# pangenome/smoothxg

Hardware: AMD Instinct MI355X
Metric: POA blocks/sec (+ DP cells/sec) on 1000-block synthetic (higher is better)
Workload: dtype int16

## Files before the change

### include/sxg_poa.h

```cpp
#ifndef SXG_POA_H
#define SXG_POA_H
#include <stdint.h>

#ifdef __cplusplus
extern "C" {
#endif

#define SXG_POA_ABI_VERSION 5

#define SXG_MODE_LOCAL 0
#define SXG_MODE_GLOBAL 1
#define SXG_ORDER_SPOA 0x10

#define SXG_OK 0
#define SXG_E_INVALID (-1)
#define SXG_E_NODEVICE (-2)
#define SXG_E_NOMEM (-3)
#define SXG_E_BLOCK (-4)
#define SXG_NOT_ROOT 1

#define SXG_ST_OK 0
#define SXG_ST_ROWS_OVERFLOW 1
#define SXG_ST_POOL_OVERFLOW 2
#define SXG_ST_TBX_OVERFLOW 3
// ... 44 lines not shown
    int32_t *edge_tail;
    int32_t *edge_head;
    uint32_t *edge_weight;
    int32_t *seq_path_nodes;
    int32_t *score;
    uint64_t *cells;
    int64_t *cons_off;
    int32_t *cons_nodes;
    int64_t *msa_off;
    int32_t *msa_cols;
    char *msa;
    int64_t *bg_node_off;
    int32_t *bg_node_len;
    int32_t *bg_node_outdeg;
    uint8_t *bg_node_indeg;
    int64_t *bg_seq_off;
    char *bg_seq;
    int64_t *bg_edge_off;
    int32_t *bg_edge_to;
    int64_t *bg_step_off;
    int32_t *bg_steps;
    int64_t *bg_cons_off;
    int32_t *bg_cons_steps;
    uint64_t *block_cycles;
    void *_owner;
} sxg_poa_batch_out;

typedef struct sxg_poa_align_in {
    int32_t n;
    const int64_t *row_off;
    const uint8_t *row_code;
    const uint8_t *row_sink;
    const int64_t *pred_off;
    const int32_t *preds;
    const int64_t *seq_off;
    const uint8_t *bases;
    const sxg_poa_params *params;
    int32_t per_problem_params;
} sxg_poa_align_in;

typedef struct sxg_poa_align_out {
    int32_t n;
    int32_t *status;
    int32_t *score;
    int64_t *pair_off;
    int32_t *pair_row;
    int32_t *pair_pos;
    void *_owner;
} sxg_poa_align_out;

typedef struct sxg_poa_stats {
    double kernel_ms;
    uint64_t cells;
    uint64_t dp_launches;
    uint64_t algo_bytes;
    int32_t n_slots;
    int32_t retries;
    uint64_t device_bytes;
    double dom_kernel_ms;
    uint64_t dom_cells, dom_algo_bytes;
    int32_t dom_threads, dom_cols_per_lane;
    int32_t dom_row_mode;
    int32_t dom_clock_mhz;
    double bg_ms;
} sxg_poa_stats;

typedef struct sxg_poa_width_stats {
    uint64_t sweeps[2];
    uint64_t swept_cols[2];
    uint64_t swept_cells[2];
    uint64_t hint_shift_repeats;
    int32_t dom_width, dom_width2;
} sxg_poa_width_stats;

typedef struct sxg_poa_twin_stats {
    uint64_t twin_steps;
    uint64_t join_rows;
} sxg_poa_twin_stats;

int sxg_poa_abi_version(void);
int sxg_poa_measure_copy(sxg_poa_handle *h, uint64_t bytes, int reps, double *gbps);
int sxg_poa_roctx_available(void);
int sxg_poa_device_count(void);
const char *sxg_poa_last_error(void);

int sxg_poa_create(int device, sxg_poa_handle **out);
void sxg_poa_destroy(sxg_poa_handle *h);

int sxg_poa_batch_run(sxg_poa_handle *h, const sxg_poa_batch_in *in, sxg_poa_batch_out *out);
int sxg_poa_batch_upload(sxg_poa_handle *h, const sxg_poa_batch_in *in);
int sxg_poa_batch_execute(sxg_poa_handle *h);
int sxg_poa_batch_download(sxg_poa_handle *h, sxg_poa_batch_out *out);
void sxg_poa_batch_free(sxg_poa_batch_out *out);

typedef struct sxg_poa_device_view {
    int32_t n_blocks;
    int64_t n_seqs, n_bases;
    const int32_t *status, *n_nodes, *n_edges;
    const uint8_t *node_code;
    const int32_t *node_rank, *node_group;
    const int32_t *edge_tail, *edge_head;
    const uint32_t *edge_weight;
    const int32_t *seq_path_nodes;
    const int32_t *score;
} sxg_poa_device_view;
int sxg_poa_batch_device_view(sxg_poa_handle *h, sxg_poa_device_view *out);

#define SXG_POA_COMM_ID_BYTES 128
int sxg_poa_comm_unique_id(uint8_t *id);
int sxg_poa_comm_init(sxg_poa_handle *h, const uint8_t *id, int nranks, int rank);
int sxg_poa_comm_attach(sxg_poa_handle *h, void *nccl_comm, int nranks, int rank);
void sxg_poa_comm_destroy(sxg_poa_handle *h);
int sxg_poa_batch_run_sharded(sxg_poa_handle *h, const sxg_poa_batch_in *in, sxg_poa_batch_out *out);
int sxg_poa_batch_upload_sharded(sxg_poa_handle *h, const sxg_poa_batch_in *in);
int sxg_poa_batch_execute_sharded(sxg_poa_handle *h);
int sxg_poa_batch_download_sharded(sxg_poa_handle *h, const sxg_poa_batch_in *in, sxg_poa_batch_out *out);
int sxg_poa_sharded_info(sxg_poa_handle *h, int32_t *ranks_seen, uint64_t *bytes_received);
int sxg_poa_sharded_timing(sxg_poa_handle *h, double *pack_ms, double *exchange_ms);
int sxg_poa_batch_run_sharded_local(sxg_poa_handle *h, const sxg_poa_batch_in *in, int nranks, sxg_poa_batch_out *out);

int sxg_poa_align_batch(sxg_poa_handle *h, const sxg_poa_align_in *in, sxg_poa_align_out *out);
void sxg_poa_align_free(sxg_poa_align_out *out);

#define SXG_POA_SPLIT_PANEL 512
int sxg_poa_pair_identity_batch(sxg_poa_handle *h, int64_t n_seqs, const int64_t *seq_off, const uint8_t *bases, int64_t n_pairs,
                                const int32_t *pair_a, const int32_t *pair_b, const uint8_t *b_rev, const int32_t *cap,
                                int32_t *penalty, int32_t *cols, int32_t *matches);
typedef struct sxg_poa_split_in {
    int32_t n_blocks;
    const int32_t *blk_off;
    const int64_t *seq_off;
    const uint8_t *bases;
    const double *identity;
    const double *length_ratio_min;
} sxg_poa_split_in;
typedef struct sxg_poa_split_out {
    int32_t n_blocks;
    int64_t n_seqs;
    int32_t *group;
    int32_t *n_groups;
    int64_t *n_pairs;
    int32_t *status;
    void *_owner;
} sxg_poa_split_out;
int sxg_poa_split_batch(sxg_poa_handle *h, const sxg_poa_split_in *in, sxg_poa_split_out *out);
void sxg_poa_split_free(sxg_poa_split_out *out);

#define SXG_POA_MASH_SORT_TILE 1024
int sxg_poa_kmer_jaccard_batch(sxg_poa_handle *h, int64_t n_seqs, const int64_t *seq_off, const uint8_t *bases, int32_t kmer_size,
                               int64_t n_pairs, const int32_t *pair_a, const int32_t *pair_b,
                               int32_t *set_size, int32_t *inter, uint64_t *kmers);
typedef struct sxg_poa_split_mash {
    int32_t kmer_size;
    const int32_t *min_len;
    const double *est_identity;
} sxg_poa_split_mash;
int sxg_poa_split_mash_batch(sxg_poa_handle *h, const sxg_poa_split_in *in, const sxg_poa_split_mash *mash,
                             sxg_poa_split_out *out, int64_t *n_mash);

typedef struct sxg_poa_identity_in {
    int32_t n_blocks; const int32_t *blk_off; const int64_t *seq_off; const uint8_t *bases;
    int32_t kmer_size;
    int32_t min_len;
    double percentile;
} sxg_poa_identity_in;
int sxg_poa_block_identity_batch(sxg_poa_handle *h, const sxg_poa_identity_in *in,
// ... 28 lines not shown
```

### smoothxg_amd/build.py

```python
import os
import subprocess

HERE = os.path.dirname(os.path.abspath(__file__))
CSRC = os.path.join(HERE, "csrc")
SO = os.path.join(CSRC, "libsxgpoa.so")
KERN_PARTS = range(1, 10)
SOURCES = [("sxg_poa.hip", "sxg_poa.o", []), ("kern_split.hip", "kern_split.o", []), ("kern_msa.hip", "kern_msa.o", []),
           ("kern_sgd.hip", "kern_sgd.o", ["-ffp-contract=off"])] + [("kern_part.hip", "kern_part%d.o" % k, ["-DSXG_KERN_PART=%d" % k]) for k in KERN_PARTS]
DEPS = ["sxg_poa.hip", "kern_part.hip", "poa_classes.h", "poa_kernels.hip.h", "poa_kern_tables.hip.h", "poa_dp.hip.h", "poa_dp16.hip.h", "poa_dp16_fill.inc.h", "poa_dp16_row.inc.h", "poa_prep_rows.inc.h", "poa_rowcode.h", "poa_band16.hip.h", "poa_graph_dev.h",
                  "poa_bgraph_dev.h", "poa_types.h", "kern_split.hip", "poa_split.hip.h", "poa_mash.hip.h", "poa_identity.hip.h", "poa_identity_key.h", "kern_sgd.hip", "poa_sgd.hip.h", "kern_msa.hip", "poa_msa.hip.h", "poa_msa_cols.h", os.path.join("..", "..", "include", "sxg_poa.h")]
OBJ_DIR = os.path.join(CSRC, "build")


def needs_build():
    if not os.path.exists(SO):
        return True
    t = os.path.getmtime(SO)
    return any(os.path.getmtime(os.path.join(CSRC, d)) > t for d in DEPS)


def build(force=False, verbose=False):
    if not force and not needs_build():
        return SO
    hipcc = os.environ.get("HIPCC", "/opt/rocm/bin/hipcc")
    flags = ["--offload-arch=gfx950", "-O3", "-std=c++17", "-fPIC"] + os.environ.get("SXG_HIPCC_FLAGS", "").split()
    os.makedirs(OBJ_DIR, exist_ok=True)
    jobs = max(1, int(os.environ.get("SXG_BUILD_JOBS", str(os.cpu_count() or 1))))
    objs, running, pending = [], [], list(SOURCES)
    failed = None
    while pending or running:
        while pending and len(running) < jobs and failed is None:
            src, obj, defs = pending.pop(0)
            obj = os.path.join(OBJ_DIR, obj)
            cmd = [hipcc] + flags + defs + ["-c", "-o", obj, os.path.join(CSRC, src)]
            if verbose:
                print(" ".join(cmd), flush=True)
            running.append((subprocess.Popen(cmd), cmd))
            objs.append(obj)
        if failed is not None:
            pending = []
        if not running:
            break
        proc, cmd = running.pop(0)
        if proc.wait() != 0 and failed is None:
            failed = cmd
    if failed is not None:
        raise subprocess.CalledProcessError(1, failed)
    cmd = [hipcc, "--offload-arch=gfx950", "-shared", "-fPIC", "-o", SO] + objs + ["-ldl"]
    if verbose:
        print(" ".join(cmd), flush=True)
    subprocess.check_call(cmd)
    return SO


SMOOTH_SO = os.path.join(CSRC, "libsxgsmooth.so")
SMOOTH_DEPS = ["sxg_smooth.cpp", "prep_host.h", os.path.join("..", "..", "include", "sxg_smooth.h"),
               os.path.join("..", "..", "include", "sxg_poa.h")]


def build_smooth(force=False, verbose=False):
    if not force and os.path.exists(SMOOTH_SO) and \
            all(os.path.getmtime(os.path.join(CSRC, d)) <= os.path.getmtime(SMOOTH_SO) for d in SMOOTH_DEPS):
        return SMOOTH_SO
    cmd = [os.environ.get("CXX", "g++"), "-O2", "-std=c++17", "-fPIC", "-shared", "-fopenmp", "-Wall", "-o", SMOOTH_SO,
           os.path.join(CSRC, "sxg_smooth.cpp")]
    if verbose:
        print(" ".join(cmd))
    subprocess.check_call(cmd)
    return SMOOTH_SO


if __name__ == "__main__":
    build(force=True, verbose=True)
    build_smooth(force=True, verbose=True)
```

### smoothxg_amd/csrc/poa_band16.hip.h

```cpp
#pragma once
#include <hip/hip_runtime.h>
#include "poa_dp16.hip.h"

namespace sxg {

constexpr int BAND_WB = 311;
constexpr double BAND_WF = 0.03;
constexpr int BAND_W_MAX = 11;
constexpr int BAND_WIN = 128;
constexpr int BAND_WMAX = 693;
__host__ __device__ inline int band_strip_width(int maxlen) {
    const int w0 = BAND_WB + (int)(BAND_WF * maxlen), w = w0 < BAND_WMAX ? w0 : BAND_WMAX;
    return 2 * w <= 756 ? 6 : (2 * w <= 1008 ? 8 : 11);
}
__host__ __device__ inline int band_half_width(int L) { const int w = BAND_WB + (int)(BAND_WF * L); return w < BAND_WMAX ? w : BAND_WMAX; }
__host__ __device__ inline int band_plane_strips(int maxlen, int W) { return plane_round4(2 * band_half_width(maxlen) / W + 2); }
__host__ __device__ constexpr int band_lds_bytes(int W) { return LDS_CTL_BYTES + LDS_META_BYTES / 2 + 64 * W * 8; }

constexpr unsigned NEGCELL = 0x0000C000u;

__device__ __forceinline__ void band_strips_of(const int hint, const int w, const int W, const int last_strip, int& bl, int& bh) {
    bl = max(hint - w, 0) / W;
    bh = min((hint + w) / W, last_strip);
}

template <bool CVX, int W, bool SW = true, int CB = 4>
__device__ __noinline__ DpResult dp_fill_band16(const Scoring S, const RowsView R, const int N_, const uint8_t* seq, const int L_,
                                               const DpBuffers B, char* smem, unsigned long long* cells_out) {
    DpResult res;
    const int N = __builtin_amdgcn_readfirstlane(N_), L = __builtin_amdgcn_readfirstlane(L_);
    const int MB = LDS_META_BYTES / 2, CH = MB / 32;
    const i32x4* lmeta = (const i32x4*)(smem + LDS_CTL_BYTES);
    const int lane = threadIdx.x;
    const int g = __builtin_amdgcn_readfirstlane(S.g), e = __builtin_amdgcn_readfirstlane(S.e);
    const int q = __builtin_amdgcn_readfirstlane(S.q), c = __builtin_amdgcn_readfirstlane(S.c);
    const int G2 = pk2(g, g), E2 = pk2(e, e), Q2 = pk2(q, q), C2 = pk2(c, c);
    const int sm = __builtin_amdgcn_readfirstlane(S.m), sn = __builtin_amdgcn_readfirstlane(S.n);
    const int NEG2 = pk2(NEGP, NEGP);
    const unsigned SC_N4 = (unsigned)(sn & 0xff) * 0x01010101u, SC_MX = (unsigned)((sm ^ sn) & 0xff);
    const int We = W * e, Wc = W * c;
    const int BS = __builtin_amdgcn_readfirstlane(B.band_strips), bw = __builtin_amdgcn_readfirstlane(B.band_w);
    const int last_strip = L / W;
    static_assert(CB == 4 || SW, "2-byte band cells: local alignment only (every cell of a band is a real score)");
    constexpr int SD = p16_slot_dwords(W, CB);
    const P16Delta DF = p16_delta_of(S);
    const int dbH_ = __builtin_amdgcn_readfirstlane(DF.bH), dbF_ = __builtin_amdgcn_readfirstlane(DF.bF);
    const int KF2 = pk2(1 << dbH_, 1 << dbH_), KO2 = pk2(1 << (dbH_ + dbF_), 1 << (dbH_ + dbF_));
    const int D_SH1 = pk2(dbH_, dbH_), D_SH2 = pk2(dbH_ + dbF_, dbH_ + dbF_);
    const int D_MH = pk2((1 << dbH_) - 1, (1 << dbH_) - 1), D_MF = pk2((1 << dbF_) - 1, (1 << dbF_) - 1);
    const int d_cst_ = g + ((-e) << dbH_) + ((CVX ? -c : 0) << (dbH_ + dbF_));
    const int D_CST = pk2(d_cst_, d_cst_);
    const int D_EA = pk2(-e, -e), D_CA = pk2(-c, -c);
    SXG_GLOBAL uint32_t* const g_tb = sxg_uniform(sxg_global((uint32_t*)B.tb));
    SXG_GLOBAL const int32_t* const g_meta = sxg_uniform(sxg_global((const int32_t*)R.meta));
    SXG_GLOBAL const int32_t* const g_preds = sxg_uniform(sxg_global((const int32_t*)R.preds));
    SXG_GLOBAL const int32_t* const g_hint = sxg_uniform(sxg_global((const int32_t*)R.tbx));
    SXG_GLOBAL const uint8_t* const g_seq = sxg_global(seq);
    const bool has_board = __builtin_amdgcn_readfirstlane((int)(B.prio_board != nullptr)) != 0;
    const int prio_rank = __builtin_amdgcn_readfirstlane(B.prio_rank);
    constexpr int NL = (W + 1) / 2;
    typedef __attribute__((address_space(3))) u32x2 lds_u32x2;
    const bool ada = __builtin_amdgcn_readfirstlane(B.band_mode) == 2;
    constexpr int REC_AUX = 0x10;
    const __amdgpu_buffer_rsrc_t rs_meta = p16_rsrc((const void*)g_meta, N * 32);
    int prev_bw = 0, prev_lr = 0;
    auto load_rec = [&](const int p) -> u32x2 {
        const u32x2 v = __builtin_amdgcn_raw_buffer_load_b64(rs_meta, 0u, (p - 1) * 32 + 24, REC_AUX);
        return u32x2{(unsigned)__builtin_amdgcn_readfirstlane((int)v.x), (unsigned)__builtin_amdgcn_readfirstlane((int)v.y)};
    };
    auto ada_band = [&](const int p_l, const int p_r, const int rem, int& bl_, int& bh_) {
        const int c_ = L - rem;
        const int b0 = max(min(p_l, c_) - bw, 0), e0 = min(max(p_r, c_) + bw, L);
        int sb = b0 / W, se = e0 / W;
        if (se - sb + 1 > BAND_WIN) {
            const int sc = min(max(c_, 0), L) / W;
            sb = max(sb, min(sc - BAND_WIN / 2, se - (BAND_WIN - 1)));
            se = sb + BAND_WIN - 1;
        }
        bl_ = sb; bh_ = se;
    };

    auto row0_h = [&](const int j) -> int {
        if (j < 0 || j > L) return NEGP;
        if (j == 0) return 0;
        const int a_ = g + (j - 1) * e, b_ = q + (j - 1) * c;
        return max(a_ > b_ ? a_ : b_, NEGP);
    };
    int s0 = -1000000;
    unsigned let[NL];
    unsigned so_lo = 0, so_hi = 0;
    int Hp[W], Fp[W], Op[W], Hleft = NEG2;
#pragma unroll
    for (int k = 0; k < W; ++k) { Hp[k] = NEG2; Fp[k] = NEG2; Op[k] = NEG2; }
    int pbl = 0, pbh = -1;
    bool regs_ok = false;
    bool next_sib = false;
    int best_lo = SW ? 0 : NEGP * 2, best_hi = best_lo, bi_lo = -1, bi_hi = -1, bj_lo = 0, bj_hi = 0;
    unsigned long long cells = 0;
// ... 472 lines not shown
```

### smoothxg_amd/csrc/poa_dp.hip.h

```cpp
#pragma once
#include <hip/hip_runtime.h>
#include "poa_types.h"

namespace sxg {

typedef unsigned u32x4 __attribute__((ext_vector_type(4)));
typedef unsigned u32x3 __attribute__((ext_vector_type(3)));

typedef __attribute__((address_space(3))) int sxg_lds_int;
template <int GBv>
struct WgCtxT {
    static constexpr int GB = GBv, GBH = GBv > 8 ? 8 : GBv, SCAN_K = GBv;
    sxg_lds_int* lds;
    __device__ __forceinline__ int tid() const { return (int)threadIdx.x; }
    __device__ __forceinline__ int nthreads() const { return (int)blockDim.x; }
    __device__ __forceinline__ void sync() const { __syncthreads(); }
    __device__ __forceinline__ int atomic_add(int32_t* p, int v) const { return atomicAdd(p, v); }
    __device__ __forceinline__ int atomic_min(int32_t* p, int v) const { return atomicMin(p, v); }
    __device__ int scan_excl_add(int v, int* total) const {
        const int lane = threadIdx.x & 63, w = threadIdx.x >> 6, nw = blockDim.x >> 6;
        int x = v;
#pragma unroll
        for (int d = 1; d < 64; d <<= 1) {
            const int o = __shfl_up(x, d);
// ... 188 lines not shown
#define SXG_PIN(...) asm volatile("" : __VA_ARGS__)
#ifndef SXG_G
#define SXG_G 1
#endif
#if SXG_G == 1
#define SXG_COLS(a, k) "+v"(a[k])
#elif SXG_G == 2
#define SXG_COLS(a, k) "+v"(a[(k) - 1]), "+v"(a[k])
#else
#define SXG_COLS(a, k) "+v"(a[(k) - 3]), "+v"(a[(k) - 2]), "+v"(a[(k) - 1]), "+v"(a[k])
#endif
#define SXG_GROUP_END(k) (((k) % SXG_G) == SXG_G - 1)

template <int W, bool CVX, bool H16, bool SW>
__device__ __forceinline__ void dp_fill(const Scoring& S, const RowsView& R, const int N,
                        const uint8_t* __restrict__ seq, const int L, const DpBuffers& B,
                        char* smem, const bool park_in_lds, const int pf_off, DpResult& res) {
    static_assert(W % 4 == 0 && W <= 24, "W must be a multiple of 4, at most 24");
    const int T = (int)blockDim.x;
    const int NW = T >> 6;
    const int Lpad = T * W;
    constexpr unsigned ALL = (1u << W) - 1u;
    using RWt = RowWord<H16>;
    using Word = typename RWt::type;
    int* lds = (int*)smem;
    const int4* lmeta = (const int4*)(smem + LDS_CTL_BYTES);
    Word* lrow = park_in_lds ? (Word*)(smem + LDS_CTL_BYTES + LDS_META_BYTES) : (Word*)B.park;
    const int t = threadIdx.x, lane = t & 63, wv = t >> 6;
    const int j0 = t * W;
    constexpr int PF_PIECES = W * (int)sizeof(Word) / 16;
    const unsigned lds_pf = (unsigned)__builtin_amdgcn_groupstaticsize() + (unsigned)(pf_off >= 0 ? pf_off : 0);
    const unsigned lds_pfl = lds_pf + (unsigned)PF_PIECES * (unsigned)T * 16u;
    int pf_row = -1;
    SXG_GLOBAL Word* const g_row0 = sxg_uniform(sxg_global((Word*)B.row0));
    SXG_GLOBAL Word* const g_pool = sxg_uniform(sxg_global((Word*)B.pool));
    SXG_GLOBAL uint8_t* const g_tb = sxg_uniform(sxg_global(B.tb));
    SXG_GLOBAL uint32_t* const g_steps = sxg_uniform(sxg_global(B.steps));
    SXG_GLOBAL const int32_t* const g_meta = sxg_uniform(sxg_global((const int32_t*)R.meta));
    SXG_GLOBAL const int32_t* const g_preds = sxg_uniform(sxg_global((const int32_t*)R.preds));
    SXG_GLOBAL const int32_t* const g_slot = sxg_uniform(sxg_global((const int32_t*)R.slot));
    const unsigned uj0 = (unsigned)(t * W);
    const int g = S.g, e = S.e, q = S.q, c = S.c, mm = S.m, mn = S.n;
    const int We = W * e, Wc = W * c;
    int* tot_a = lds;
    int* tot_b = lds + 16;
    int* xch_h = lds + 32;
    int* xch_b = lds + 48;

    unsigned qcw[W / 4];
#pragma unroll
    for (int k4 = 0; k4 < W / 4; ++k4) {
        unsigned v = 0;
#pragma unroll
        for (int b = 0; b < 4; ++b) {
            const int j = j0 + k4 * 4 + b;
            const unsigned ch = (j >= 1 && j <= L) ? (unsigned)seq[j - 1] : 255u;
            v |= (ch > 4u && ch != 255u ? 4u : ch) << (8 * b);
        }
        qcw[k4] = v;
    }

    int Hp[W], Fp[W], Op[W], Hleft;
#pragma unroll
    for (int k = 0; k < W; ++k) {
        const int j = j0 + k;
        int h = 0;
        if (!SW && j > 0) { const int a = g + (j - 1) * e, b = q + (j - 1) * c; h = a > b ? a : b; }
        Hp[k] = h; Fp[k] = NEG; Op[k] = NEG;
    }
    {
        const int j = j0 - 1;
        int h = 0;
        if (!SW && j > 0) { const int a = g + (j - 1) * e, b = q + (j - 1) * c; h = a > b ? a : b; }
        Hleft = j < 0 ? NEG : h;
    }
    {
#pragma unroll
        for (int k = 0; k < W; ++k) (g_row0 + k)[uj0] = RWt::pack(Hp[k], Fp[k], Op[k]);
    }
    int best = SW ? 0 : NEG * 2, bi = -1, bj = -1;
    const int kL = L - j0;

    for (int i = 1; i <= N; ++i) {
        if (B.prio_board) { if ((i & 127) == 1) sxg_balance_prio(B, (unsigned long long)i * (unsigned long long)L); }
        else if ((i & 63) == 1) sxg_rotate_prio(B.prio_rank);
        const int r = i - 1;
        if ((r & (META_CHUNK - 1)) == 0) {
            __syncthreads();
            SXG_GLOBAL const i32x4* gm = (SXG_GLOBAL const i32x4*)(g_meta + 8 * (size_t)r);
            i32x4* lm = (i32x4*)(smem + LDS_CTL_BYTES);
            const int nrow = min(META_CHUNK, N - r);
            for (int x = t; x < 2 * nrow; x += T) lm[x] = gm[x];
            __syncthreads();
        }
        const int4 m0 = lmeta[2 * (r & (META_CHUNK - 1))], m1 = lmeta[2 * (r & (META_CHUNK - 1)) + 1];
        const int pb = __builtin_amdgcn_readfirstlane(m0.x);
        const int info = __builtin_amdgcn_readfirstlane(m0.y);
        const int p0 = __builtin_amdgcn_readfirstlane(m0.z);
        const int s0 = __builtin_amdgcn_readfirstlane(m0.w);
        const int p1 = __builtin_amdgcn_readfirstlane(m1.x);
        const int s1 = __builtin_amdgcn_readfirstlane(m1.y);
        const int myslot = __builtin_amdgcn_readfirstlane(m1.z);
        const int tx = __builtin_amdgcn_readfirstlane(m1.w);
        const int np = info & 0xffff, code = (info >> 16) & 0xff, flags = (info >> 24) & 0xff;
#pragma unroll
        for (int k4 = 0; k4 < W / 4; ++k4) SXG_PIN("+v"(qcw[k4]));

        int Hc[W];
        unsigned fxm = 0, oxm = 0;

#define SXG_READ_PF(wr, hl)                                                                    \
    do {                                                                                       \
        asm volatile("s_waitcnt vmcnt(0)" ::: "memory");                                       \
        _Pragma("unroll") for (int c_ = 0; c_ < PF_PIECES; ++c_) {                             \
            const u32x4 v_ = *(const __attribute__((address_space(3))) u32x4*)(size_t)(lds_pf + (unsigned)c_ * (unsigned)T * 16u + (unsigned)t * 16u); \
            if (H16) {                                                                         \
                *(unsigned*)&wr[4 * c_] = v_.x; *(unsigned*)&wr[4 * c_ + 1] = v_.y;            \
                *(unsigned*)&wr[4 * c_ + 2] = v_.z; *(unsigned*)&wr[4 * c_ + 3] = v_.w;        \
            } else {                                                                           \
                *(uint2*)&wr[2 * c_] = make_uint2(v_.x, v_.y);                                 \
                *(uint2*)&wr[2 * c_ + 1] = make_uint2(v_.z, v_.w);                             \
            }                                                                                  \
        }                                                                                      \
        const unsigned l_ = *(const __attribute__((address_space(3))) unsigned*)(size_t)(lds_pfl + (unsigned)t * 4u); \
        hl = j0 > 0 ? (H16 ? (int)(short)(l_ & 0xffffu) : (int)l_) : NEG;                      \
    } while (0)
#define SXG_INIT(k, hs, fs, os, hprev)                                              \
    do {                                                                            \
        const int c1_ = (hs) + g, c2_ = (fs) + e;                                   \
        const bool x1_ = c2_ > c1_;                                                 \
        const int d1_ = (hs) + q, d2_ = (os) + c;                                   \
        const bool x2_ = CVX && d2_ > d1_;                                          \
        Hc[k] = (hprev);                                                            \
        Fp[k] = x1_ ? c2_ : c1_;                                                    \
        fxm |= (unsigned)x1_ << (k);                                                \
        if (CVX) { Op[k] = x2_ ? d2_ : d1_; oxm |= (unsigned)x2_ << (k); }          \
    } while (0)
#define SXG_PIN_INIT(k) \
    if (SXG_GROUP_END(k)) SXG_PIN(SXG_COLS(Hc, k), SXG_COLS(Fp, k), SXG_COLS(Op, k), "+v"(fxm), "+v"(oxm))

        if (np <= 1 && p0 == i - 1) {
#pragma unroll
            for (int k = 0; k < W; ++k) {
                SXG_INIT(k, Hp[k], Fp[k], Op[k], (k ? Hp[k - 1] : Hleft));
                SXG_PIN_INIT(k);
            }
        } else {
            const bool reg0 = (p0 == i - 1), reg1 = (np == 2 && p1 == i - 1);
            const bool park = np >= 3;
            if (park) {
#pragma unroll
                for (int k = 0; k < W; ++k) lrow[j0 + k] = RWt::pack(Hp[k], Fp[k], Op[k]);
            }
            const int ge = reg1 ? 1 : 0;
            if ((reg0 || reg1) && !park) {
#pragma unroll
                for (int k = 0; k < W; ++k) {
                    SXG_INIT(k, Hp[k], Fp[k], Op[k], (k ? Hp[k - 1] : Hleft));
                    SXG_PIN_INIT(k);
                }
            } else {
                Word wr[W];
                int hl = Hleft;
                if (reg0) {
#pragma unroll
                    for (int k = 0; k < W; ++k) wr[k] = lrow[j0 + k];
                } else if (p0 == pf_row) {
// ... 274 lines not shown
```

### smoothxg_amd/csrc/poa_dp16_fill.inc.h

```cpp
    DpResult res;
    const int N = __builtin_amdgcn_readfirstlane(N_), L = __builtin_amdgcn_readfirstlane(L_);
    static_assert(W >= 4 && W <= 15, "strip width");
    const int T = TFIX ? TFIX : (int)blockDim.x;
    constexpr bool ONEW = TFIX == 64;
    const int NW = T >> 6;
    const int TW = T * W;
    const int MB = dp16_meta_bytes(T);
    int* lds = (int*)smem;
    const int t = threadIdx.x, lane = t & 63, wv = ONEW ? 0 : __builtin_amdgcn_readfirstlane(t >> 6);
    const int s_lo = wv * 128 + 2 * lane, s_hi = s_lo + 1;
    const int j0 = s_lo * W, j0h = s_hi * W;
    const int g = DS ? P16_DEF_G : __builtin_amdgcn_readfirstlane(S.g), e = DS ? P16_DEF_E : __builtin_amdgcn_readfirstlane(S.e);
    const int q = DS ? P16_DEF_Q : __builtin_amdgcn_readfirstlane(S.q), c = DS ? P16_DEF_C : __builtin_amdgcn_readfirstlane(S.c);
    const int sm = DS ? P16_DEF_M : __builtin_amdgcn_readfirstlane(S.m), sn = DS ? P16_DEF_N : __builtin_amdgcn_readfirstlane(S.n);
    const int G2 = pk2(g, g), E2 = pk2(e, e), Q2 = pk2(q, q), C2 = pk2(c, c);
    constexpr int BIAS = SW ? P16_BIAS : 0, FLOORV = SW ? P16_FLOOR : NEGP;
    const int NEG2 = pk2(FLOORV, FLOORV), B2 = pk2(BIAS, BIAS), NWF2 = pk2(P16_NWFLOOR, P16_NWFLOOR);
    const unsigned Gm = (unsigned)(-g) * 0x10001u, Em = (unsigned)(-e) * 0x10001u, Qm = (unsigned)(-q) * 0x10001u, Cm = (unsigned)(-c) * 0x10001u;
#define P16_DEC(x, Km, K2) (SW ? (int)((unsigned)(x) - (Km)) : pk_add((x), (K2)))
#define P16_INC(x, Km, K2) (SW ? (int)((unsigned)(x) + (Km)) : pk_sub((x), (K2)))
    const unsigned SC_N4 = (unsigned)(sn & 0xff) * 0x01010101u, SC_MX = (unsigned)((sm ^ sn) & 0xff);
    const int We = W * e, Wc = W * c;
    const int BS = __builtin_amdgcn_readfirstlane(B.band_strips);
    constexpr int SD = p16_slot_dwords(W, CB);
// ... 65 lines not shown
    {
        int h2[2];
#pragma unroll
        for (int hf = 0; hf < 2; ++hf) {
            const int j = (hf ? j0h : j0) - 1;
            int h = BIAS;
            if (!SW && j > 0) { const int a = g + (j - 1) * e, b = q + (j - 1) * c; h = max(a > b ? a : b, P16_NWFLOOR); }
            h2[hf] = j < 0 ? FLOORV : h;
        }
        Hleft = pk2(h2[0], h2[1]);
    }
    {
        const __amdgpu_buffer_rsrc_t rs0 = p16_rsrc((const void*)g_row0, RB);
        if constexpr (CB == 2) {
            const int lh0 = t == 0 ? (int)(((unsigned)Hleft & 0xffff0000u) | ((unsigned)Hp[0] & 0x0000ffffu)) : Hleft;
            int prev = lh0;
#pragma unroll
            for (int k = 0; k < W; ++k) {
                __builtin_amdgcn_raw_buffer_store_b32((unsigned)p16_row_encode<CVX, SW>(Hp[k], prev, Fp[k], Op[k], DFu, RC), rs0, (unsigned)t * 4u, k * T * 4, 0);
                prev = Hp[k];
            }
            __builtin_amdgcn_raw_buffer_store_b32((unsigned)lh0, rs0, (unsigned)t * 4u, TW * 4, 0);
        } else {
#pragma unroll
            for (int k = 0; k < W; ++k)
                __builtin_amdgcn_raw_buffer_store_b64(p16_pack_row<CVX, SW>(Hp[k], Fp[k], Op[k]), rs0, ut8, k * T * 8, 0);
            __builtin_amdgcn_raw_buffer_store_b32((unsigned)Hleft, rs0, (unsigned)t * 4u, TW * 8, 0);
        }
    }
    int best_lo = NEGP * 2, best_hi = best_lo, bi_lo = -1, bi_hi = -1, bk_lo = 0, bk_hi = 0;
    const int kL_lo = L - j0, kL_hi = L - j0h;
    unsigned key_lo = 0u, key_hi = 0u;
    unsigned long long ekey = 0ull;
    auto fold_keys = [&](const int i_end) {
        const unsigned ep = (unsigned)(i_end - 1) >> 16;
        auto k64 = [&](const unsigned k, const int strip) -> unsigned long long {
            if (k == 0u) return 0ull;
            const unsigned row = (ep << 16) | (0xffffu - (k & 0xffffu));
            return ((unsigned long long)(k >> 16) << 32) | ((unsigned long long)(0xFFFFFu - row) << 12) | (unsigned long long)(0xFFFu - (unsigned)strip);
        };
        unsigned long long kk = k64(key_lo, s_lo);
        const unsigned long long k2 = k64(key_hi, s_hi);
        kk = k2 > kk ? k2 : kk;
#pragma unroll
        for (int d = 32; d >= 1; d >>= 1) {
            const unsigned long long o = __shfl_xor(kk, d);
            kk = o > kk ? o : kk;
        }
        const unsigned hi_ = (unsigned)__builtin_amdgcn_readfirstlane((int)(kk >> 32)), lo_ = (unsigned)__builtin_amdgcn_readfirstlane((int)kk);
        const unsigned long long ku = ((unsigned long long)hi_ << 32) | lo_;
        ekey = ku > ekey ? ku : ekey;
        key_lo = 0u; key_hi = 0u;
    };

    typedef __attribute__((address_space(3))) u32x2 lds_u32x2;
    const unsigned lds_rows0 = lds0 + (unsigned)(LDS_CTL_BYTES + MB);
#define P16_LDS_ROW(words_, left_, b_)                                                                      \
    int tq_ = t;                                                                                            \
    asm volatile("" : "+v"(tq_));                                                                           \
    const unsigned lb_ = lds_rows0 + (unsigned)(b_) * (unsigned)RB;                                         \
    std::conditional_t<CB == 2, lds_u32, lds_u32x2>* const words_ = (std::conditional_t<CB == 2, lds_u32, lds_u32x2>*)(size_t)(lb_ + (unsigned)(wv * (64 * RWB * W - 64 * RWB)) + (unsigned)tq_ * (unsigned)RWB); \
    lds_u32* const left_ = (lds_u32*)(size_t)(lb_ + (unsigned)(TW * RWB) + (unsigned)tq_ * 4u)
    const bool has_board = __builtin_amdgcn_readfirstlane((int)(B.prio_board != nullptr)) != 0;
    const unsigned soff = (unsigned)(s_lo % BS) | ((unsigned)(s_hi % BS) << 16);
    const int prio_rank = __builtin_amdgcn_readfirstlane(B.prio_rank);
#ifdef SXG_ROW_PROF
#define P16_PROF_FETCH() do { RP_MARK(0); asm volatile("s_waitcnt vmcnt(0)" ::: "memory"); RP_MARK(6); } while (0)
#else
#define P16_PROF_FETCH() do { } while (0)
#endif
#ifdef SXG_ROW_PROF
    unsigned long long racc[8] = {0};
#define RP_MARK(seg) do { const unsigned long long tn_ = __builtin_readcyclecounter(); racc[seg] += tn_ - rt_; rt_ = tn_; } while (0)
#else
#define RP_MARK(seg) do { } while (0)
#endif
    typedef int i32x8 __attribute__((ext_vector_type(8)));
    typedef __attribute__((address_space(4))) const i32x8 const_i32x8;
    const_i32x8* const cmeta = (const_i32x8*)(unsigned long long)g_meta;
    __builtin_amdgcn_s_dcache_inv();
    i32x8 dnext = cmeta[0];
    if constexpr (TWIN) { const int d1_ = dnext[1]; asm volatile("" :: "s"(d1_)); }
    for (int i = 1; i <= N; ++i) {
        if (has_board) { if ((i & 127) == 1) sxg_balance_prio(B, (unsigned long long)i * (unsigned long long)L); }
        else if ((i & 63) == 1) sxg_rotate_prio(prio_rank);
        i32x8 dsc = dnext;
        dnext = cmeta[min(i, N - 1)];
        int pb = dsc[0], info = dsc[1], p0 = dsc[2], s0 = dsc[3], p1 = dsc[4], s1 = dsc[5], myslot = dsc[6], hint = dsc[7];
        int np = info & 0xffff, code = (info >> 16) & 0xff, flags = (info >> 24) & 0xff;
        unsigned SC_T0 = SC_N4 ^ (code < 4 ? SC_MX << (8 * code) : 0u), SC_T1 = SC_N4 ^ (code == 4 ? SC_MX : 0u);

#ifdef SXG_ROW_PROF
        unsigned long long rt_ = __builtin_readcyclecounter();
#endif
        int Hc[W];
#define P16_FETCH(p_, sl_, wr_, hl_)                                                                        \
    do {                                                                                                    \
        if ((sl_) <= -2) {                                                                                  \
            P16_LDS_ROW(la_, lf_, -2 - (sl_));                                                              \
            _Pragma("unroll") for (int k = 0; k < W; ++k) wr_[k] = la_[k * 64];                             \
            hl_ = (int)*lf_;                                                                                \
        } else {                                                                                            \
            const __amdgpu_buffer_rsrc_t rs_ = p16_rsrc(((p_) == 0) ? (const void*)g_row0 : (const void*)((SXG_GLOBAL const char*)g_pool + (size_t)(sl_) * (size_t)RB), RB); \
            if constexpr (CB == 2) {                                                                        \
                _Pragma("unroll") for (int k = 0; k < W; ++k) wr_[k] = __builtin_amdgcn_raw_buffer_load_b32(rs_, ut8 >> 1, k * T * 4, 0); \
            } else {                                                                                        \
                _Pragma("unroll") for (int k = 0; k < W; ++k) wr_[k] = __builtin_amdgcn_raw_buffer_load_b64(rs_, ut8, k * T * 8, 0); \
            }                                                                                               \
            P16_PROF_FETCH();                                                                               \
            hl_ = (int)__builtin_amdgcn_raw_buffer_load_b32(rs_, ut8 >> 1, TW * RWB, 0);                     \
            P16_DRAIN();                                                                                    \
        }                                                                                                   \
    } while (0)
#define P16_DECODE(wr_, hl_, HS_, FS_, OS_)                                                                 \
    do {                                                                                                    \
        int run_ = hl_;                                                                                     \
        _Pragma("unroll") for (int k = 0; k < W; ++k) {                                                     \
            p16_row_decode<CVX, SW>(wr_[k], run_, FS_[k], OS_[k], RC);                                      \
            HS_[k] = run_;                                                                                  \
        }                                                                                                   \
        if (t == 0) hl_ = (int)(((unsigned)hl_ & 0xffff0000u) | ((unsigned)FLOORV & 0xffffu));               \
    } while (0)

#define P16_FETCH_PLANE(p_, HS_, FS_, OS_, hl_)                                                             \
    do {                                                                                                    \
        const __amdgpu_buffer_rsrc_t rsp_ = p16_rsrc((const void*)(g_tb + (size_t)(p_) * (size_t)(SD * BS)), SD * BS * 4); \
        unsigned dl_[SD], dh_[SD];                                                                          \
        plane_load_strip<SD>(rsp_, soff & 0xffffu, BS, dl_);                                                \
        plane_load_strip<SD>(rsp_, soff >> 16, BS, dh_);                                                    \
        P16_PROF_FETCH();                                                                                   \
        P16_DRAIN();                                                                                        \
        int run_ = (int)__builtin_amdgcn_perm(dh_[0], dl_[0], 0x05040100u);                                 \
        hl_ = t == 0 ? (int)(((unsigned)run_ & 0xffff0000u) | ((unsigned)FLOORV & 0xffffu)) : run_;         \
        _Pragma("unroll") for (int k = 0; k < W; ++k) {                                                     \
            const unsigned cn_ = __builtin_amdgcn_perm(dh_[(k + 1) >> 1], dl_[(k + 1) >> 1], ((k + 1) & 1) ? 0x07060302u : 0x05040100u); \
            p16_row_decode<CVX, SW>(cn_, run_, FS_[k], OS_[k], RC);                                         \
            HS_[k] = run_;                                                                                  \
        }                                                                                                   \
    } while (0)

#define P16_DRAIN() __builtin_amdgcn_s_waitcnt(0x0F70)
        if constexpr (TWIN) {
            bool swept_out = false;
            while (flags & ROW_TWIN) {
                if (has_board) {
                    const int due = ((i + 1) & 127) == 1 ? i + 1 : ((((i + 2) & 127) == 1 && i + 2 <= N) ? i + 2 : 0);
                    if (due) sxg_balance_prio(B, (unsigned long long)due * (unsigned long long)L);
                } else if (((i + 1) & 63) == 1 || (((i + 2) & 63) == 1 && i + 2 <= N)) sxg_rotate_prio(prio_rank);
                if (p0 != i - 1) {
                    int hl;
                    unsigned wr[W];
                    P16_FETCH(p0, s0, wr, hl);
                    P16_DECODE(wr, hl, Hp, Fp, Op);
#pragma unroll
                    for (int k = 0; k < W; ++k) SXG_PIN("+v"(Hp[k]), "+v"(Fp[k]), "+v"(Op[k]));
                    Hleft = hl;
                }
                if (!CVX) {
#pragma unroll
                    for (int k = 0; k < W; ++k) Op[k] = NEG2;
                }
                const i32x8 dsc2 = dnext;
                dnext = cmeta[min(i + 1, N - 1)];
                const int i2 = i + 1;
                const int info2 = dsc2[1], cd2 = (info2 >> 16) & 0xff;
                const unsigned t0_2 = SC_N4 ^ (cd2 < 4 ? SC_MX << (8 * cd2) : 0u), t1_2 = SC_N4 ^ (cd2 == 4 ? SC_MX : 0u);
                int Hc2[W], a2, b2, HLB;
#define P16_ROW_MODE 1
#define P16_ROW_PART 1
#include "poa_dp16_row.inc.h"
#undef P16_ROW_PART
                {
                    const unsigned SC_T0 = t0_2, SC_T1 = t1_2;
                    int (&Hc)[W] = Hc2;
#define P16_ROW_PART 1
#include "poa_dp16_row.inc.h"
#undef P16_ROW_PART
                    a2 = a; b2 = b;
                }
                {
#define P16_ROW_PART 2
#include "poa_dp16_row.inc.h"
#undef P16_ROW_PART
                }
#undef P16_ROW_MODE
                {
                    const bool twin_joined = (((dnext[1] >> 24) & 0xff) & ROW_JOIN) != 0;
                    const int fl2 = (info2 >> 24) & 0xff, ms2 = dsc2[6], hn2 = dsc2[7];
                    int (&HB)[W] = Hc;
                    {
                        const int i = i2, flags = fl2, myslot = ms2, hint = hn2;
                        const unsigned SC_T0 = t0_2, SC_T1 = t1_2;
                        int (&Hc)[W] = Hc2;
                        int a = a2, b = b2;
#define P16_ROW_MODE 2
#define P16_ROW_PART 2
#include "poa_dp16_row.inc.h"
#undef P16_ROW_PART
#undef P16_ROW_MODE
                    }
                }
                i += 2;
                if (i > N) { swept_out = true; break; }
                dsc = dnext;
                dnext = cmeta[min(i, N - 1)];
                pb = dsc[0]; info = dsc[1]; p0 = dsc[2]; s0 = dsc[3]; p1 = dsc[4]; s1 = dsc[5]; myslot = dsc[6]; hint = dsc[7];
                np = info & 0xffff; code = (info >> 16) & 0xff; flags = (info >> 24) & 0xff;
                SC_T0 = SC_N4 ^ (code < 4 ? SC_MX << (8 * code) : 0u); SC_T1 = SC_N4 ^ (code == 4 ? SC_MX : 0u);
            }
            if (swept_out) break;
        }
        if ((EXP & 32) || (np <= 1 && p0 == i - 1)) {
        } else {
            const bool regbase = (flags & ROW_REGPRED) != 0;
            bool joinrow = false;
            if constexpr (TWIN) joinrow = (flags & ROW_JOIN) != 0;
#define P16_NOT_PAIR(p_) (!TWIN || !joinrow || (p_) != i - 2)
            if (!regbase) {
                int hl;
                if (ring_plane && s0 >= 0 && p0 != 0) P16_FETCH_PLANE(p0, Hp, Fp, Op, hl);
                else if constexpr (CB == 2) {
                    unsigned wr[W];
                    P16_FETCH(p0, s0, wr, hl);
                    P16_DECODE(wr, hl, Hp, Fp, Op);
#pragma unroll
                    for (int k = 0; k < W; ++k) SXG_PIN("+v"(Hp[k]), "+v"(Fp[k]), "+v"(Op[k]));
                } else {
                    u32x2 wr[W];
                    P16_FETCH(p0, s0, wr, hl);
#pragma unroll
// ... 116 lines not shown
```

### smoothxg_amd/csrc/poa_kernels.hip.h

```cpp
#pragma once
#include <hip/hip_runtime.h>
#include <algorithm>
#include <cstdlib>
#include <cstring>

#include "../../include/sxg_poa.h"
#include "poa_classes.h"
#include "poa_dp.hip.h"
#include "poa_dp16.hip.h"
#include "poa_band16.hip.h"
#include "poa_graph_dev.h"
#include "poa_bgraph_dev.h"

using namespace sxg;


struct SlotLayout {
    size_t hdr, code, rank, order, order_tmp, leader, gmem, in_head, in_tail, out_head, out_tail, in_deg,
        out_deg, e_tail, e_head, e_next_in, e_next_out, e_w, posnode, target, newidx, nexta, preva, slotadd,
        kind, xpos, via, dfs_stack, dfs_rec, sp_rank, sp_first, sp_cnt, r_code, r_flags, r_pred_off, r_preds, r_slot, r_tbx, r_sseq, r_row_node, r_meta, tb, steps, pool,
        row0, park, cons_sc, cons_pr, pair_row, pair_pos, total;
    int nodes_cap, rows_cap, pool_slots, step_cap, scratch_len, Lpad, word_bytes, threads;
    int band_strips;
    int lds_rows;
// ... 65 lines not shown
        return std::min(plane_round4((cols + W - 1) / W), 2 * T);
    }
    return p16_band_strips(T, W);
}

inline bool width2_enabled() {
    const char* e = getenv("SXG_POA_WIDTH2");
    return !(e && atoi(e) == 0);
}

struct P16LaunchSizes { int strips, strips2, lds_rows, smem; };
inline P16LaunchSizes p16_launch_sizes(int T, int W, int W2, int CB, bool wide_band) {
    P16LaunchSizes s;
    s.strips = wide_band ? 2 * T : plane_strips_p16(T, W);
    s.strips2 = W2 ? (wide_band ? 2 * T : plane_strips_p16(T, W2)) : 0;
    s.lds_rows = p16_lds_rows(T, W, CB);
    s.smem = std::max(dp16_lds_bytes(T, W, s.lds_rows, CB), W2 ? dp16_lds_bytes(T, W2, s.lds_rows, CB) : 0);
    return s;
}

struct SlotViews {
    GraphView G;
    RowsView R;
    DpBuffers B;
    int64_t* cons_sc;
    int32_t* cons_pr;
    int32_t *pair_row, *pair_pos;
};

__device__ static SlotViews slot_views(uint8_t* base, const SlotLayout& L) {
    SlotViews V;
    SXG_GP int32_t* hdr = (SXG_GP int32_t*)(base + L.hdr);
    V.G.n_nodes = hdr; V.G.n_edges = hdr + 1;
    V.G.code = (SXG_GP uint8_t*)(base + L.code);
#define P32(f) (SXG_GP int32_t*)(base + L.f)
    V.G.rank = P32(rank); V.G.order = P32(order); V.G.order_tmp = P32(order_tmp); V.G.leader = P32(leader);
    V.G.gmem = P32(gmem); V.G.in_head = P32(in_head); V.G.in_tail = P32(in_tail); V.G.out_head = P32(out_head);
    V.G.out_tail = P32(out_tail); V.G.in_deg = P32(in_deg); V.G.out_deg = P32(out_deg);
    V.G.e_tail = P32(e_tail); V.G.e_head = P32(e_head); V.G.e_next_in = P32(e_next_in);
    V.G.e_next_out = P32(e_next_out); V.G.e_w = (SXG_GP uint32_t*)(base + L.e_w);
    V.G.posnode = P32(posnode); V.G.target = P32(target); V.G.newidx = P32(newidx); V.G.nexta = P32(nexta);
    V.G.preva = P32(preva); V.G.slotadd = P32(slotadd); V.G.kind = (SXG_GP int8_t*)(base + L.kind);
    V.G.xpos = P32(xpos); V.G.via = P32(via); V.G.dfs_stack = P32(dfs_stack); V.G.dfs_rec = P32(dfs_rec);
    V.G.sp_rank = P32(sp_rank); V.G.sp_first = P32(sp_first); V.G.sp_cnt = P32(sp_cnt);
    V.R.code = (SXG_GP uint8_t*)(base + L.r_code); V.R.flags = (SXG_GP uint8_t*)(base + L.r_flags); V.R.pred_off = P32(r_pred_off);
    V.R.preds = P32(r_preds); V.R.slot = P32(r_slot); V.R.tbx = P32(r_tbx); V.R.sseq = P32(r_sseq);
    V.R.row_node = P32(r_row_node); V.R.meta = P32(r_meta);
    V.B.tb = base + L.tb; V.B.steps = (uint32_t*)(base + L.steps);
    V.B.pool = base + L.pool; V.B.row0 = base + L.row0; V.B.park = base + L.park;
    V.B.band_strips = L.band_strips; V.B.lds_rows = L.lds_rows;
    V.cons_sc = (int64_t*)(base + L.cons_sc); V.cons_pr = (int32_t*)(base + L.cons_pr);
    V.pair_row = (int32_t*)(base + L.pair_row); V.pair_pos = (int32_t*)(base + L.pair_pos);
#undef P32
    return V;
}

__host__ __device__ static inline Scoring normalise(const sxg_poa_params& p) {
    Scoring S;
    S.m = p.m; S.n = p.n; S.g = p.g; S.e = p.e; S.q = p.q; S.c = p.c;
    S.sw = (p.mode & 1) == SXG_MODE_LOCAL;
    S.convex = 0;
    if (S.g >= S.e) { S.e = S.g; S.q = S.g; S.c = S.g; }
    else if (S.g <= S.q || S.e >= S.c) { S.q = S.g; S.c = S.e; }
    else S.convex = 1;
    return S;
}

struct BlockArgs {
    const int32_t* blk_off; const int64_t* seq_off; const uint8_t* bases; const uint32_t* weights;
    const sxg_poa_params* params; int per_block_params;
    const int32_t* work; int n_work; int32_t* queue;
    uint8_t* arena; SlotLayout lay;
    int32_t* status; int32_t* n_nodes; int32_t* n_edges; int32_t* n_cons;
    uint8_t* node_code; int32_t* node_rank; int32_t* node_group;
    int32_t* edge_tail; int32_t* edge_head; uint32_t* edge_weight;
    int32_t* paths; int32_t* score; unsigned long long* cells; int32_t* cons_nodes;
    int want_consensus;
    int park_in_lds;
    int pf_off;
    int num_cu;
    uint32_t* prio_board;
    int prio_base;
    const unsigned long long* est;
    int lds_bytes;
    unsigned long long* blk_cycles;
    int band_floor, band_margin, band_full;
    int twin;
};

__host__ __device__ constexpr int sxg_min_waves(int TMAX, int W, int RM) { return class_traits(TMAX, W, RM, 4).min_waves; }

template <int TMAX, int W, bool CVX, int RM, bool SW, int CB = 4, bool DS = false, int W2 = 0>
__global__ __launch_bounds__(TMAX, sxg_min_waves(TMAX, W, RM)) void poa_block_kernel(const BlockArgs A) {
    static_assert(W2 == 0 || (RM == 2 && W2 < W), "a second strip width: packed sweep, narrower than the first");
    constexpr bool H16 = RM != 1;
    constexpr int CPL = RM >= 2 ? 2 * W : W;
    constexpr ClassTraits CT = class_traits(TMAX, W, RM, CB);
    const int T = (int)blockDim.x;
    extern __shared__ __attribute__((aligned(16))) char smem[];
    int* lds = (int*)smem;
    int& s_work = lds[200];
    WgCtx ctx{(sxg_lds_int*)(size_t)((unsigned)__builtin_amdgcn_groupstaticsize() + 128u * 4u)};
    const int t = threadIdx.x;
    SlotViews V = slot_views(A.arena + (size_t)blockIdx.x * A.lay.total, A.lay);
    V.B.prio_rank = (int)(blockIdx.x / (unsigned)A.num_cu + (unsigned)A.prio_base) & (PRIO_BOARD_SLOTS - 1);
    V.B.prio_board = A.prio_board ? A.prio_board + (size_t)(__smid() & (PRIO_BOARD_CUS - 1)) * PRIO_BOARD_SLOTS : nullptr;
    const RowCaps caps{A.lay.rows_cap, A.lay.pool_slots, A.lay.step_cap, A.lay.lds_rows};
    bool first = true;
    for (;;) {
        __syncthreads();
        if (t == 0) s_work = first ? (int)blockIdx.x : (int)gridDim.x + atomicAdd(A.queue, 1);
        first = false;
        __syncthreads();
        const int wi = s_work;
        if (wi >= A.n_work) break;
        const int b = A.work[wi];
        const unsigned long long est_total = A.est ? A.est[wi] : 0ull;
        unsigned long long done_cells = 0;
        const int s0 = A.blk_off[b], s1 = A.blk_off[b + 1];
        const int64_t base0 = A.seq_off[s0];
        const Scoring S = normalise(A.params[A.per_block_params ? b : 0]);
        if (t == 0) { *V.G.n_nodes = 0; *V.G.n_edges = 0; }
        __syncthreads();
        int status = ST_OK;
        unsigned long long* prof = (unsigned long long*)(A.arena + (size_t)blockIdx.x * A.lay.total + A.lay.hdr + 64);
        V.B.row_prof = prof + 28;
        if ((t & 63) == 0) {
            prof[10 + (t >> 6)] = ((unsigned long long)__smid() << 32) | (unsigned long long)__builtin_amdgcn_s_getreg(GETREG_IMMED(31, 0, HW_ID));
            if (t == 0 && prof[8] == 0) { prof[8] = (unsigned long long)wall_clock64(); prof[6] = (unsigned long long)clock64(); }
        }
        unsigned long long tc0 = clock64(), tc1;
        const unsigned long long tblk0 = tc0;
        int band_drift = 0, band_min = 0;
#define PROF(k) do { if (t == 0) { tc1 = clock64(); prof[k] += tc1 - tc0; tc0 = tc1; } } while (0)
        for (int s = s0; s < s1 && status == ST_OK; ++s) {
            const int64_t so = A.seq_off[s];
            const int len = (int)(A.seq_off[s + 1] - so);
            const uint8_t* seq = A.bases + so;
            for (int i = t; i < len; i += T) V.G.posnode[i] = -1;
            __syncthreads();
            const int N = *V.G.n_nodes;
            int score = 0;
            if (RM != 3 && len + 1 > T * CPL) { status = ST_TOO_LONG; break; }
            if (N + len > A.lay.nodes_cap || *V.G.n_edges + len > A.lay.nodes_cap) { status = ST_NODES_OVERFLOW; break; }
            if (RM != 1 && RM != 2 && !S.sw &&
                -(sxg_gap_cost(S.g, S.e, S.q, S.c, N) + sxg_gap_cost(S.g, S.e, S.q, S.c, len)) >= (RM >= 2 ? 15800 : 30000)) {
                status = ST_RANGE_OVERFLOW;
                break;
            }
            if (N > 0 && len > 0) {
                PROF(0);
                const int band_mode = RM == 3 ? (int)A.params[A.per_block_params ? b : 0].banded : 0;
                const int hinted_ = RM == 3 ? (band_mode == 2 ? 3 : 2) : (RM == 2 ? 1 : 0);
                if constexpr (RM == 2 && CT.twin != 0) {
                    static_assert(CT.graph_batch == 4, "twin classes: the plain workgroup context");
                    unsigned long long n2 = 0;
                    status = prep_rows_twin(ctx, V.G, V.R, caps, hinted_, A.twin, &n2);
                    if (status == ST_OK && n2) atomicAdd(&prof[55], n2);
                }
                else if (CT.graph_batch == 16 || (CT.graph_batch == 8 && T <= 64)) { WgCtxT<16> c16{ctx.lds}; status = prep_rows(c16, V.G, V.R, caps, hinted_); }
                else if (CT.graph_batch == 8) { WgCtxT<8> c8{ctx.lds}; status = prep_rows(c8, V.G, V.R, caps, hinted_); }
                else status = prep_rows(ctx, V.G, V.R, caps, hinted_);
                if (status != ST_OK) break;
                PROF(1);
                DpResult res;
                V.B.prio_rem0 = est_total > done_cells ? est_total - done_cells : 0ull;
                if constexpr (RM == 3) {
                    V.B.band_w = band_half_width(len);
                    V.B.band_mode = band_mode;
                    res = dp_fill_band16<CVX, W, SW, SW ? CB : 4>(S, V.R, N, seq, len, V.B, smem, A.cells + s);
                    __syncthreads();
                    PROF(2);
                    if (t == 0) lds[TBM_FLAG] = 0;
                    __syncthreads();
                    if (res.bi >= 0)
                        traceback_p16<false, W, CVX, true, SW ? CB : 4>(V.R, V.B, S, seq, len, res.best, T, min(256, (len << 8) / max(N, 1)), res.bi, res.bj,
                                                                        V.G.posnode, nullptr, nullptr, smem);
                    __syncthreads();
                    PROF(3);
                    if (lds[TBM_FLAG]) { status = ST_INTERNAL; break; }
                } else if constexpr (RM == 2) {
                    auto sweep = [&](auto wk_) {
                        constexpr int Wk = decltype(wk_)::value;
                        constexpr int narrow = Wk != W ? 1 : 0;
                        const int bs_cap = narrow ? A.lay.band_strips2 : A.lay.band_strips;
                        int bs = bs_cap;
                        if (A.band_floor > 0 && bs_cap < 2 * T && s - s0 > A.band_full)
                            bs = max(p16_drift_strips(band_drift, A.band_margin, Wk, A.band_floor, bs_cap), min(plane_round4((band_min + Wk - 1) / Wk), bs_cap));
                        for (int att = 0;; ++att) {
                            V.B.band_strips = bs;
                            if (t == 0) {
                                prof[47] += (unsigned long long)bs; prof[48] += 1;
                                prof[49 + narrow] += 1; prof[51 + narrow] += (unsigned long long)(T * 2 * Wk); prof[53 + narrow] += (unsigned long long)N * (unsigned long long)(T * 2 * Wk);
                            }
#ifdef SXG_EXP
                            if (att == 0) { res = dp_fill_p16<Wk, CVX, SW, CB, CT.rp, CT.tfix, DS, SXG_EXP>(S, V.R, N, seq, len, V.B, smem); __syncthreads(); if (res.best == 0x7fffffff) break; }
#endif
                            if constexpr (CT.twin != 0) res = dp_fill_p16_twin<Wk, CVX, SW, CB, CT.rp, CT.tfix, DS>(S, V.R, N, seq, len, V.B, smem);
                            else res = dp_fill_p16<Wk, CVX, SW, CB, CT.rp, CT.tfix, DS>(S, V.R, N, seq, len, V.B, smem);
                            __syncthreads();
                            PROF(2);
                            if (t == 0) { lds[TBM_FLAG] = 0; lds[TBM_RANGE] = 0; }
                            __syncthreads();
                            if (t < 64 && res.bi >= 0)
                                traceback_p16<false, Wk, CVX, false, CB>(V.R, V.B, S, seq, len, res.best, T, min(256, (len << 8) / max(N, 1)), res.bi, res.bj,
                                                                         V.G.posnode, nullptr, nullptr, smem);
                            __syncthreads();
                            PROF(3);
                            if (lds[TBM_RANGE]) { status = ST_RANGE_OVERFLOW; break; }
                            if (!lds[TBM_FLAG]) break;
                            if (att == 5) { status = ST_BAND_MISS; break; }
                            const int mrow = lds[TBM_ROW], mdelta = lds[TBM_DELTA];
                            __syncthreads();
                            for (int r2 = t; r2 < mrow; r2 += T) V.R.meta[8 * (size_t)r2 + 7] += mdelta;
                            for (int i2 = t; i2 < len; i2 += T) V.G.posnode[i2] = -1;
                            if (t == 0) prof[27] += 1;
                            bs = min(plane_round4(2 * bs), bs_cap);
                            band_min = bs * Wk;
                            __syncthreads();
                        }
                        if (status != ST_OK) return;
                        if (A.band_floor > 0 && bs_cap < 2 * T) {
                            int d = 0;
                            for (int j2 = t; j2 < len; j2 += T) {
                                const int v = V.G.posnode[j2];
                                if (v >= 0) d = max(d, abs(j2 + 1 - V.G.xpos[v]));
                            }
                            band_drift = max(band_drift, ctx.reduce_max(d));
                        }
                    };
                    if constexpr (W2 != 0) {
                        if (width_for_len(W, A.lay.W2, T, len) != W) sweep(std::integral_constant<int, W2>{});
                        else sweep(std::integral_constant<int, W>{});
                    } else sweep(std::integral_constant<int, W>{});
                    if (status != ST_OK) break;
                } else {
                    dp_fill<W, CVX, H16, SW>(S, V.R, N, seq, len, V.B, smem, A.park_in_lds != 0, A.pf_off, res);
                    __syncthreads();
                    PROF(2);
                    if (t == 0 && res.bi >= 0) traceback<false>(V.R, V.B, T, W, S.sw, res.bi, res.bj, V.G.posnode, nullptr, nullptr);
                    __syncthreads();
                    PROF(3);
                }
                score = res.bi >= 0 ? res.best : 0;
            }
            if (t == 0) { A.score[s] = score; if (RM != 3 || N == 0 || len == 0) A.cells[s] = RM == 3 ? 0ull : (unsigned long long)N * (unsigned long long)len; }
            done_cells += (unsigned long long)N * (unsigned long long)len;
            const bool spoa_order = (A.params[A.per_block_params ? b : 0].mode & SXG_ORDER_SPOA) != 0;
            if (CT.graph_batch == 16 || (CT.graph_batch == 8 && T <= 64)) { WgCtxT<16> c16{ctx.lds}; add_alignment(c16, V.G, seq, len, A.weights ? A.weights[s] : 1u, A.paths + so, !spoa_order); }
            else if (CT.graph_batch == 8) { WgCtxT<8> c8{ctx.lds}; add_alignment(c8, V.G, seq, len, A.weights ? A.weights[s] : 1u, A.paths + so, !spoa_order); }
            else add_alignment(ctx, V.G, seq, len, A.weights ? A.weights[s] : 1u, A.paths + so, !spoa_order);
            if (spoa_order) {
                typedef __attribute__((address_space(3))) uint8_t lds_u8;
                spoa_resort(ctx, V.G, (lds_u8*)(size_t)((unsigned)__builtin_amdgcn_groupstaticsize() + (unsigned)LDS_CTL_BYTES), A.lds_bytes - LDS_CTL_BYTES,
                            (int)(A.seq_off[s0 + 1] - A.seq_off[s0]), len, N, s == s0, prof + 41);
                __syncthreads();
            }
            PROF(4);
        }
        PROF(0);
        __syncthreads();
        const int N = *V.G.n_nodes, E = *V.G.n_edges;
        if (status == ST_OK) {
            for (int v = t; v < N; v += T) {
                A.node_code[base0 + v] = V.G.code[v];
                A.node_rank[base0 + v] = V.G.rank[v];
                A.node_group[base0 + v] = V.G.leader[v];
            }
            for (int e = t; e < E; e += T) {
                A.edge_tail[base0 + e] = V.G.e_tail[e];
                A.edge_head[base0 + e] = V.G.e_head[e];
                A.edge_weight[base0 + e] = V.G.e_w[e];
            }
            int nc = 0;
            if (A.want_consensus && t == 0) nc = consensus_serial(V.G, V.cons_sc, V.cons_pr, A.cons_nodes + base0);
            if (t == 0) { A.n_nodes[b] = N; A.n_edges[b] = E; A.n_cons[b] = nc; }
        } else if (t == 0) { A.n_nodes[b] = 0; A.n_edges[b] = 0; A.n_cons[b] = 0; }
        if (t == 0) { A.status[b] = status; if (A.blk_cycles) A.blk_cycles[b] = (unsigned long long)clock64() - tblk0; }
        if (t == 0 && V.B.prio_board) __hip_atomic_store(V.B.prio_board + V.B.prio_rank, 0u, __ATOMIC_RELAXED, __HIP_MEMORY_SCOPE_AGENT);
        PROF(5);
        if (t == 0) { prof[9] = (unsigned long long)wall_clock64(); prof[7] = (unsigned long long)clock64(); }
#undef PROF
    }
}

struct AlignArgs {
    const int64_t* row_off; const uint8_t* row_code; const uint8_t* row_sink; const int64_t* pred_off;
    const int32_t* preds; const int64_t* seq_off; const uint8_t* bases; const sxg_poa_params* params;
    int per_problem_params;
    const int32_t* work; int n_work; int32_t* queue;
    uint8_t* arena; SlotLayout lay;
    int32_t* status; int32_t* score; int32_t* n_pairs;
    int32_t* pair_row; int32_t* pair_pos;
    int park_in_lds;
    int pf_off;
    int num_cu;
};

template <int TMAX, int W, bool CVX, int RM, bool SW>
__global__ __launch_bounds__(TMAX, sxg_min_waves(TMAX, W, RM)) void poa_align_kernel(const AlignArgs A) {
    constexpr bool H16 = RM != 1;
    constexpr int CPL = RM == 2 ? 2 * W : W;
    const int T = (int)blockDim.x;
    extern __shared__ __attribute__((aligned(16))) char smem[];
    int* lds = (int*)smem;
    int& s_work = lds[200];
    WgCtx ctx{(sxg_lds_int*)(size_t)((unsigned)__builtin_amdgcn_groupstaticsize() + 128u * 4u)};
    const int t = threadIdx.x;
    SlotViews V = slot_views(A.arena + (size_t)blockIdx.x * A.lay.total, A.lay);
    V.B.prio_rank = (int)(blockIdx.x / (unsigned)A.num_cu) & (PRIO_BOARD_SLOTS - 1);
    V.B.prio_board = nullptr; V.B.prio_rem0 = 0; V.B.row_prof = nullptr;
    const RowCaps caps{A.lay.rows_cap, A.lay.pool_slots, A.lay.step_cap, A.lay.lds_rows};
    for (;;) {
        __syncthreads();
        if (t == 0) s_work = atomicAdd(A.queue, 1);
        __syncthreads();
        const int wi = s_work;
        if (wi >= A.n_work) break;
        const int p = A.work[wi];
        const int64_t r0 = A.row_off[p];
        const int N = (int)(A.row_off[p + 1] - r0);
        const int64_t so = A.seq_off[p];
        const int len = (int)(A.seq_off[p + 1] - so);
        const Scoring S = normalise(A.params[A.per_problem_params ? p : 0]);
        const int64_t e0 = A.pred_off[r0];
        int status = ST_OK, score = 0, npairs = 0;
        if (len + 1 > T * CPL) status = ST_TOO_LONG;
        else if (N > A.lay.rows_cap) status = ST_ROWS_OVERFLOW;
        else if (N > 0 && len > 0) {
            for (int r = t; r < N; r += T) {
// ... 51 lines not shown
```

### smoothxg_amd/csrc/sxg_poa.hip

```cpp
#include <hip/hip_runtime.h>
#include <algorithm>
#include <chrono>
#include <cmath>
#include <cstdio>
#include <cstdlib>
#include <cstring>
#include <memory>
#include <new>
#include <string>
#include <sys/mman.h>
#include <thread>
#include <vector>

#include "../../include/sxg_poa.h"
#include <rccl/rccl.h>
#include <dlfcn.h>
#include "poa_kernels.hip.h"
#include "poa_kern_tables.hip.h"
#include "poa_split.hip.h"
#include "poa_mash.hip.h"
#include "poa_identity.hip.h"
#include "poa_sgd.hip.h"
#include "poa_msa.hip.h"


struct BgArgs {
    const int32_t* blk_off; const int64_t* seq_off; const uint8_t* bases; const int32_t* paths;
    const uint8_t* node_code; const int32_t* edge_tail; const int32_t* edge_head; const int32_t* cons;
    const int32_t *nn, *ne, *nc; const int32_t* trim; int cons_mode;
    const int32_t* work; int n_work; int32_t* queue;
    uint8_t* arena; size_t slot_bytes; int capV, capE, capC, capT;
    const int64_t *node_o, *edge_o;
    int32_t *o_len, *o_outdeg; uint8_t* o_indeg; char* o_seq; int32_t* o_eto; int32_t* o_steps; int32_t* o_nsteps;
    int32_t* o_cons; int32_t* o_counts;
};
constexpr int BG_THREADS = 256, BG_HEAP = 3072;
static size_t bg_slot_bytes(int capV, int capE, int capC, int capT) {
    return 4 * (27 * ((size_t)capV + 2) + 3 * ((size_t)capE + capC + 2) + ((size_t)capC + 2) + ((size_t)capT + 2) + 4) + 256;
}
struct BgCtx : WgCtx {
    int* hp;
    __device__ __forceinline__ int load_fresh(const int32_t* p) const { return __hip_atomic_load(p, __ATOMIC_RELAXED, __HIP_MEMORY_SCOPE_AGENT); }
    __device__ __forceinline__ int* heap() const { return hp; }
    __device__ __forceinline__ int heap_cap() const { return BG_HEAP; }
};
__global__ __launch_bounds__(BG_THREADS) void block_graph_kernel(const BgArgs A) {
    __shared__ int s_scan[64];
    __shared__ int s_heap[BG_HEAP];
    __shared__ int s_work;
    BgCtx ctx;
    ctx.lds = (sxg_lds_int*)s_scan;
    ctx.hp = s_heap;
    const int t = threadIdx.x;
    int32_t* w = (int32_t*)(A.arena + (size_t)blockIdx.x * A.slot_bytes);
    const size_t C = (size_t)A.capV + 2, EC = (size_t)A.capE + A.capC + 2;
    BgScratch W;
    auto take = [&](size_t n) { int32_t* q = w; w += n; return q; };
    W.vis = take(C); W.front = take(C); W.back = take(C); W.ecnt = take(C); W.eoff = take(C);
    W.ehead = take(EC); W.eused = take(EC);
    W.outdeg = take(C); W.indeg = take(C); W.only = take(C); W.nxt = take(C); W.prv = take(C);
    W.pj0 = take(C); W.pj1 = take(C); W.pd0 = take(C); W.pd1 = take(C); W.cid = take(C);
    W.head_of = take(C); W.tail_of = take(C); W.clen = take(C); W.indc = take(C); W.coff = take(C); W.newid = take(C);
    W.csucc = take(EC); W.cc = take((size_t)A.capC + 2); W.tmp = take((size_t)A.capT + 2);
    W.lenN = take(C); W.odN = take(C); W.soffN = take(C); W.eoffN = take(C); W.flag = take(4);
    for (;;) {
        __syncthreads();
        if (t == 0) s_work = atomicAdd(A.queue, 1);
        __syncthreads();
        const int wi = s_work;
        if (wi >= A.n_work) break;
        const int b = A.work[wi];
        const int s0 = A.blk_off[b], s1 = A.blk_off[b + 1];
        const int64_t base0 = A.seq_off[s0];
        BgIn I;
        I.node_code = A.node_code + base0; I.V = A.nn[b]; I.E = A.ne[b];
        I.e_tail = A.edge_tail + base0; I.e_head = A.edge_head + base0;
        I.paths = A.paths + base0; I.bases = A.bases + base0; I.seq_off = A.seq_off; I.s0 = s0; I.s1 = s1;
        I.trim = A.trim ? A.trim[b] : 0;
        I.cons = A.cons ? A.cons + base0 : nullptr; I.n_cons = A.cons ? A.nc[b] : 0; I.cons_mode = A.cons ? A.cons_mode : 0;
        BgOut O;
        const int64_t no = A.node_o[b], eo = A.edge_o[b];
        O.node_len = A.o_len + no; O.node_outdeg = A.o_outdeg + no; O.node_indeg = A.o_indeg + no; O.seq = A.o_seq + no;
        O.eto = A.o_eto + eo; O.steps = A.o_steps + base0; O.nsteps = A.o_nsteps + s0; O.cons_steps = A.o_cons + no;
        O.counts = A.o_counts + (size_t)BGC_N * b;
        block_graph(ctx, I, W, O);
    }
}

__global__ void clamp_bases_kernel(uint8_t* bases, const int64_t n) {
    const int64_t n16 = (n + 15) / 16;
    for (int64_t i = (int64_t)blockIdx.x * blockDim.x + threadIdx.x; i < n16; i += (int64_t)gridDim.x * blockDim.x) {
        u32x4 v = ((const u32x4*)bases)[i];
        unsigned w[4] = {v.x, v.y, v.z, v.w};
        bool any = false;
#pragma unroll
        for (int k = 0; k < 4; ++k) {
            unsigned o = 0;
#pragma unroll
            for (int b = 0; b < 4; ++b) { const unsigned c = (w[k] >> (8 * b)) & 0xffu; o |= (c > 4u ? 4u : c) << (8 * b); }
            any |= o != w[k];
// ... 89 lines not shown
        if (e != hipSuccess) {
            want = bytes;
            e = hipMalloc(&p, want);
        }
        if (e != hipSuccess) { p = nullptr; return fail(SXG_E_NOMEM, "hipMalloc failed for " + std::to_string(bytes) + " bytes"); }
        cap = want;
        return SXG_OK;
    }
    void release() { if (p) (void)hipFree(p); p = nullptr; cap = 0; }
    template <class Tp> Tp* as() const { return (Tp*)p; }
};

struct BlockMeta {
    int maxlen = 0, nseq = 0, rm = 0; bool fits = false; Variant variant{16, 1, 256, 0};
    int tier = 0;
    bool wide_band = false;
    bool no_wide = false;
    int64_t sumlen = 0;
    double cost = 0;
    bool cvx = false, sw = true;
    Scoring S;
};

static void classify_block(BlockMeta& m, int at_least, bool clamp_ok) {
    m.rm = row_mode(m.S, m.maxlen, m.maxlen, at_least, clamp_ok);
    const int cb = m.rm == 2 ? plane_cell_bytes(m.S) : 4;
    int fw, fnw;
    forced_p16(&fw, &fnw);
    m.fits = variant_for_len(m.maxlen, m.rm, &m.variant, m.S.sw, cb, fw, fnw);
    m.variant.CB = cb;
    m.variant.DS = m.rm == 2 && cb == 2 && p16_default_scores(m.S) && !getenv("SXG_POA_NO_DEFAULT_CLASS");
}

struct PlanRes {
    DevBuf arena, work, queue, est;
    hipStream_t stream = nullptr;
    hipEvent_t e0 = nullptr, e1 = nullptr;
};

struct PinPool {
    struct Buf { void* p; size_t cap; bool busy; };
    std::mutex mu;
    std::vector<Buf> bufs;
    void* acquire(size_t bytes) {
        std::lock_guard<std::mutex> g(mu);
        for (auto& b : bufs) if (!b.busy && b.cap >= bytes) { b.busy = true; return b.p; }
        for (size_t i = 0; i < bufs.size(); ++i)
            if (!bufs[i].busy) { (void)hipHostFree(bufs[i].p); bufs.erase(bufs.begin() + (long)i); break; }
        if (bufs.size() >= 4) return nullptr;
        void* q = nullptr;
        const size_t cap = bytes + bytes / 8;
        if (hipHostMalloc(&q, cap, hipHostMallocDefault) != hipSuccess || !q) { (void)hipGetLastError(); return nullptr; }
        bufs.push_back(Buf{q, cap, true});
        return q;
    }
    void release(void* p) {
        std::lock_guard<std::mutex> g(mu);
        for (auto& b : bufs) if (b.p == p) b.busy = false;
    }
    void prewarm(size_t bytes) { if (void* p = acquire(bytes)) release(p); }
    ~PinPool() { for (auto& b : bufs) (void)hipHostFree(b.p); }
};
struct sxg_poa_handle {
    std::vector<PlanRes*> planres;
    int device = 0;
    hipStream_t stream = nullptr;
    hipEvent_t ev0 = nullptr, ev1 = nullptr;
    int num_cu = 256;
    uint64_t mem_budget = 0;
    bool have_batch = false, executed = false;
    int n_blocks = 0;
    int64_t n_seqs = 0, n_bases = 0;
    int want_consensus = 0, want_msa = 0, per_block_params = 0;
    std::vector<int32_t> h_blk_off;
    std::vector<int64_t> h_seq_off;
    std::vector<sxg_poa_params> h_params;
    std::vector<BlockMeta> meta;
    DevBuf d_blk_off, d_seq_off, d_bases, d_weights, d_params;
    bool has_weights = false;
    DevBuf d_status, d_nn, d_ne, d_nc, d_node_code, d_node_rank, d_node_group, d_edge_tail, d_edge_head, d_edge_w,
        d_paths, d_score, d_cells, d_cons, d_work, d_queue, d_arena, d_blk_cycles;
    DevBuf d_tmp_a, d_tmp_b, d_tmp_c, d_tmp_d;
    DevBuf d_board;
    int want_block_graph = 0, bg_cons_visited_only = 0;
    std::shared_ptr<PinPool> pins;
    std::thread pin_thread;
    bool bg_done = false;
    DevBuf d_trim, d_bg_no, d_bg_eo, d_bg_len, d_bg_od, d_bg_id, d_bg_seq, d_bg_eto, d_bg_steps, d_bg_nsteps, d_bg_cons, d_bg_counts,
        d_bg_work, d_bg_queue, d_bg_arena;
    std::vector<int64_t> bg_node_o, bg_edge_o;
    std::vector<int32_t> bg_counts;
    bool msa_done = false;
    DevBuf d_msa_no, d_msa_tmp, d_msa_col, d_msa_be, d_msa_off, d_msa_items, d_msa_work, d_msa_queue, d_msa;
    std::vector<int64_t> msa_off_h;
    std::vector<int32_t> d_trim_h;
    std::vector<int32_t> msa_cols_h;
    double msa_cols_ms = 0, msa_rows_ms = 0;
    sxg_poa_stats stats{};
    sxg_poa_width_stats wstats{};
    sxg_poa_twin_stats tstats{};
    ncclComm_t comm = nullptr;
    bool own_comm = false;
    int nranks = 1, rank = 0;
    DevBuf d_blob, d_recv, d_counts;
    std::vector<std::vector<int32_t>> sh_parts;
    std::vector<int64_t> sh_counts;
    std::vector<size_t> sh_at;
    bool sh_dealt = false, sh_exchanged = false;
    uint64_t sh_bytes_received = 0;
    int sh_ranks_seen = 0;
    double sh_pack_ms = 0, sh_exchange_ms = 0;
};

namespace {
struct Roctx {
    int (*push)(const char*) = nullptr;
    int (*pop)() = nullptr;
    Roctx() {
        if (getenv("SXG_POA_NO_ROCTX")) return;
        void* lib = dlopen("librocprofiler-sdk-roctx.so", RTLD_NOW | RTLD_GLOBAL);
        if (!lib) lib = dlopen("librocprofiler-sdk-roctx.so.1", RTLD_NOW | RTLD_GLOBAL);
        if (!lib) lib = dlopen("libroctx64.so", RTLD_NOW | RTLD_GLOBAL);
        if (!lib) lib = dlopen("libroctx64.so.4", RTLD_NOW | RTLD_GLOBAL);
        if (!lib) return;
        push = (int (*)(const char*))dlsym(lib, "roctxRangePushA");
        pop = (int (*)())dlsym(lib, "roctxRangePop");
        if (!push || !pop) { push = nullptr; pop = nullptr; }
    }
};
static Roctx& roctx() { static Roctx r; return r; }
struct RoctxRange {
    bool on;
    explicit RoctxRange(const char* name) : on(roctx().push != nullptr) { if (on) roctx().push(name); }
    ~RoctxRange() { if (on) roctx().pop(); }
    RoctxRange(const RoctxRange&) = delete;
    RoctxRange& operator=(const RoctxRange&) = delete;
};
}
extern "C" int sxg_poa_roctx_available(void) { return roctx().push != nullptr ? 1 : 0; }

__global__ __launch_bounds__(256) void sxg_copy_kernel(const u32x4* __restrict__ src, u32x4* __restrict__ dst, const size_t n16) {
    const size_t stride = (size_t)gridDim.x * blockDim.x;
    for (size_t i = (size_t)blockIdx.x * blockDim.x + threadIdx.x; i < n16; i += stride)
        __builtin_nontemporal_store(__builtin_nontemporal_load(src + i), dst + i);
}
extern "C" int sxg_poa_measure_copy(sxg_poa_handle* h, uint64_t bytes, int reps, double* gbps) {
    if (!h || !gbps) return fail(SXG_E_INVALID, "NULL argument");
    *gbps = 0;
    HIPCHK(hipSetDevice(h->device));
    const size_t n16 = (size_t)std::max<uint64_t>(bytes, 1u << 20) / 16;
    DevBuf a, b;
    if (int rc = a.ensure(n16 * 16)) return rc;
    if (int rc = b.ensure(n16 * 16)) return rc;
    HIPCHK(hipMemsetAsync(a.p, 1, n16 * 16, h->stream));
    hipEvent_t e0, e1;
    HIPCHK(hipEventCreate(&e0)); HIPCHK(hipEventCreate(&e1));
    const int grid = std::max(h->num_cu, 1) * 16;
    reps = std::max(reps, 1);
    hipLaunchKernelGGL(sxg_copy_kernel, dim3((unsigned)grid), dim3(256), 0, h->stream, a.as<u32x4>(), b.as<u32x4>(), n16);
    HIPCHK(hipEventRecord(e0, h->stream));
    for (int r = 0; r < reps; ++r)
        hipLaunchKernelGGL(sxg_copy_kernel, dim3((unsigned)grid), dim3(256), 0, h->stream, a.as<u32x4>(), b.as<u32x4>(), n16);
    HIPCHK(hipEventRecord(e1, h->stream));
    HIPCHK(hipEventSynchronize(e1));
    float ms = 0;
    HIPCHK(hipEventElapsedTime(&ms, e0, e1));
    (void)hipEventDestroy(e0); (void)hipEventDestroy(e1);
    a.release(); b.release();
    if (ms > 0) *gbps = 2.0 * (double)(n16 * 16) * reps / ((double)ms * 1e-3) / 1e9;
    return SXG_OK;
}

extern "C" int sxg_poa_abi_version(void) { return SXG_POA_ABI_VERSION; }
extern "C" const char* sxg_poa_last_error(void) {
    if (!g_err.empty()) return g_err.c_str();
    { std::lock_guard<std::mutex> lk(g_err_mu); g_err_ret = g_err_any; }
    return g_err_ret.c_str();
}
extern "C" int sxg_poa_device_count(void) {
    int n = 0;
    if (hipGetDeviceCount(&n) != hipSuccess) return 0;
    return n;
}

extern "C" int sxg_poa_create(int device, sxg_poa_handle** out) {
    if (!out) return fail(SXG_E_INVALID, "out is NULL");
    *out = nullptr;
    setenv("GPU_MAX_HW_QUEUES", "16", 0);
    int n = 0;
    if (hipGetDeviceCount(&n) != hipSuccess || n <= 0) return fail(SXG_E_NODEVICE, "no HIP device available");
    if (device < 0 || device >= n) return fail(SXG_E_INVALID, "device index out of range");
    HIPCHK(hipSetDevice(device));
    sxg_poa_handle* h = new sxg_poa_handle();
    h->device = device;
    h->pins = std::make_shared<PinPool>();
    hipDeviceProp_t prop;
    HIPCHK(hipGetDeviceProperties(&prop, device));
    h->num_cu = prop.multiProcessorCount;
    HIPCHK(hipStreamCreateWithFlags(&h->stream, hipStreamNonBlocking));
    HIPCHK(hipEventCreate(&h->ev0));
    HIPCHK(hipEventCreate(&h->ev1));
    *out = h;
    return SXG_OK;
}

static void release_all(sxg_poa_handle* h) {
    DevBuf* bufs[] = {&h->d_blk_off, &h->d_seq_off, &h->d_bases, &h->d_weights, &h->d_params, &h->d_status, &h->d_nn,
                      &h->d_ne, &h->d_nc, &h->d_node_code, &h->d_node_rank, &h->d_node_group, &h->d_edge_tail,
                      &h->d_edge_head, &h->d_edge_w, &h->d_paths, &h->d_score, &h->d_cells, &h->d_cons, &h->d_work,
                      &h->d_queue, &h->d_arena, &h->d_blk_cycles, &h->d_tmp_a, &h->d_tmp_b, &h->d_tmp_c, &h->d_tmp_d, &h->d_board, &h->d_trim, &h->d_bg_no, &h->d_bg_eo,
                      &h->d_bg_len, &h->d_bg_od, &h->d_bg_id, &h->d_bg_seq, &h->d_bg_eto, &h->d_bg_steps, &h->d_bg_nsteps, &h->d_bg_cons,
                      &h->d_bg_counts, &h->d_bg_work, &h->d_bg_queue, &h->d_bg_arena,
                      &h->d_msa_no, &h->d_msa_tmp, &h->d_msa_col, &h->d_msa_be, &h->d_msa_off, &h->d_msa_items, &h->d_msa_work, &h->d_msa_queue, &h->d_msa};
    for (DevBuf* b : bufs) b->release();
}

extern "C" void sxg_poa_comm_destroy(sxg_poa_handle* h);
extern "C" void sxg_poa_destroy(sxg_poa_handle* h) {
    if (!h) return;
    if (h->pin_thread.joinable()) h->pin_thread.join();
    (void)hipSetDevice(h->device);
    sxg_poa_comm_destroy(h);
    h->d_blob.release(); h->d_recv.release(); h->d_counts.release();
    release_all(h);
    for (PlanRes* r : h->planres) {
        r->arena.release(); r->work.release(); r->queue.release(); r->est.release();
        if (r->e0) (void)hipEventDestroy(r->e0);
        if (r->e1) (void)hipEventDestroy(r->e1);
        if (r->stream) (void)hipStreamDestroy(r->stream);
        delete r;
    }
    if (h->ev0) (void)hipEventDestroy(h->ev0);
    if (h->ev1) (void)hipEventDestroy(h->ev1);
    if (h->stream) (void)hipStreamDestroy(h->stream);
    delete h;
}

extern "C" int sxg_poa_set_memory_budget(sxg_poa_handle* h, uint64_t bytes) {
    if (!h) return fail(SXG_E_INVALID, "handle is NULL");
    h->mem_budget = bytes;
    return SXG_OK;
}

extern "C" int sxg_poa_get_stats(sxg_poa_handle* h, sxg_poa_stats* out) {
    if (!h || !out) return fail(SXG_E_INVALID, "NULL argument");
    *out = h->stats;
    return SXG_OK;
}

extern "C" int sxg_poa_get_width_stats(sxg_poa_handle* h, sxg_poa_width_stats* out) {
    if (!h || !out) return fail(SXG_E_INVALID, "NULL argument");
    *out = h->wstats;
    return SXG_OK;
}

extern "C" int sxg_poa_get_twin_stats(sxg_poa_handle* h, sxg_poa_twin_stats* out) {
    if (!h || !out) return fail(SXG_E_INVALID, "NULL argument");
    *out = h->tstats;
    return SXG_OK;
}

static bool twin_enabled() {
    const char* e = getenv("SXG_POA_TWIN");
    return !(e && atoi(e) == 0);
}

static uint64_t arena_budget(sxg_poa_handle* h) {
    size_t fr = 0, tot = 0;
    if (hipMemGetInfo(&fr, &tot) != hipSuccess) return 8ull << 30;
    uint64_t avail = (uint64_t)fr + h->d_arena.cap;
    for (PlanRes* r : h->planres) avail += r->arena.cap;
    uint64_t b = avail / 4 * 3;
    if (h->mem_budget && h->mem_budget < b) b = h->mem_budget;
    return b;
}

extern "C" int sxg_poa_batch_upload(sxg_poa_handle* h, const sxg_poa_batch_in* in) {
    if (!h || !in) return fail(SXG_E_INVALID, "NULL argument");
    if (in->n_blocks < 0 || (in->n_blocks > 0 && (!in->blk_off || !in->seq_off || !in->params)))
        return fail(SXG_E_INVALID, "batch_in has NULL arrays");
    HIPCHK(hipSetDevice(h->device));
    const RoctxRange range_("sxg_poa_batch_upload");
    HostLaps laps;
    h->have_batch = false; h->executed = false;
    const int nb = in->n_blocks;
    if (nb > 0 && in->blk_off[0] != 0) return fail(SXG_E_INVALID, "blk_off[0] must be 0");
    const int64_t ns = nb ? in->blk_off[nb] : 0;
    for (int b = 0; b < nb; ++b)
        if (in->blk_off[b + 1] < in->blk_off[b]) return fail(SXG_E_INVALID, "blk_off not monotone");
    if (ns > 0 && in->seq_off[0] != 0) return fail(SXG_E_INVALID, "seq_off[0] must be 0");
    for (int64_t s = 0; s < ns; ++s)
        if (in->seq_off[s + 1] < in->seq_off[s]) return fail(SXG_E_INVALID, "seq_off not monotone");
    const int64_t nbases = ns ? in->seq_off[ns] : 0;
// ... 103 lines not shown
        if (k >= 2) A.band_margin = std::max(m, 0);
        if (k >= 3) A.band_full = std::max(n, 0);
    }
}

static void prepare_plan(sxg_poa_handle* h, LaunchPlan& P, int attempt) {
    const Variant V = P.variant;
    const int Lpad = V.Lpad();
    int nodes_cap = 0, maxlen = 0;
    bool any_adaptive = false;
    bool any_spoa = false;
    double rows_est = 0;
    for (int b : P.work) {
        const BlockMeta& m = h->meta[b];
        any_adaptive = any_adaptive || h->h_params[h->per_block_params ? b : 0].banded == 2;
        any_spoa = any_spoa || (h->h_params[h->per_block_params ? b : 0].mode & SXG_ORDER_SPOA) != 0;
        nodes_cap = (int)std::max<int64_t>(nodes_cap, m.sumlen);
        maxlen = std::max(maxlen, m.maxlen);
        rows_est = std::max(rows_est, (double)m.maxlen * std::max(2.0, 1.0 + 0.0165 * m.nseq));
    }
    nodes_cap += 8;
    const int nodes_full = nodes_cap;
    int rows_cap, pool_slots, step_cap;
    if (attempt == 0) {
        rows_cap = (int)std::min<double>(nodes_cap, rows_est + 1024);
        pool_slots = std::min(rows_cap + 1, 768);
        step_cap = rows_cap;
        nodes_cap = (int)std::min<int64_t>(nodes_full, 2LL * rows_cap + maxlen + 8);
    } else if (attempt == 1) {
        rows_cap = (int)std::min<double>(nodes_cap, 2.5 * rows_est + 4096);
        pool_slots = std::min(rows_cap + 1, 4096);
        step_cap = 3 * rows_cap;
        nodes_cap = (int)std::min<int64_t>(nodes_full, 2LL * rows_cap + maxlen + 8);
    } else if (attempt == 2) {
        rows_cap = nodes_cap; pool_slots = std::min(rows_cap + 1, 32768); step_cap = nodes_cap;
    } else {
        rows_cap = nodes_cap; pool_slots = rows_cap + 1; step_cap = nodes_cap;
    }
    if (rows_cap >= (1 << 20)) rows_cap = (1 << 20) - 1;
    const int wb = V.RM == 1 ? 8 : 4;
    if (V.RM == 3) pool_slots = 1;
    const int strips1 = V.RM == 3 ? (any_adaptive ? BAND_WIN : band_plane_strips(maxlen, V.W)) : (V.RM == 2 ? p16_launch_sizes(V.T(), V.W, 0, V.CB, P.wide_band).strips : 0);
    P.variant.TMAX = class_tmax(V.W, V.NW, V.RM, V.CB, strips1 == 2 * V.T());
    P.variant.W2 = width2_enabled() ? class_w2(CLASS_BLOCK, P.variant, P.sw) : 0;
    const P16LaunchSizes LS = p16_launch_sizes(V.T(), V.W, P.variant.W2, V.CB, P.wide_band);
    P.lay = make_layout(nodes_cap, rows_cap, pool_slots, step_cap, V.T(), Lpad, wb, false, strips1, V.RM >= 2 ? V.CB : 4, any_spoa,
                        V.RM == 2 ? P.variant.W2 : 0, LS.strips2);
    P.kern = block_kernel(P.variant, P.cvx, P.sw);
    const int tfix = class_traits(P.variant.TMAX, V.W, V.RM, V.CB).tfix;
    if (tfix && tfix != V.T()) { P.kern = nullptr; P.why = "kernel class compiled for " + std::to_string(tfix) + " threads asked to run at " + std::to_string(V.T()); }
    if (!P.kern && P.why.empty()) P.why = "no kernel class built for this geometry";
    P.smem = dp_lds_launch_bytes(Lpad, wb);
    P.park_lds = dp_park_in_lds(Lpad, wb);
    if (V.RM == 2) { P.lay.lds_rows = LS.lds_rows; P.smem = LS.smem; P.park_lds = true; }
    if (V.RM == 3) { P.smem = band_lds_bytes(V.W); P.park_lds = true; }
    P.pf_off = (V.RM < 2 && getenv("SXG_POA_PREFETCH")) ? dp_pf_offset(Lpad, wb, V.T()) : -1;
    if (P.pf_off >= 0) P.smem += dp_pf_bytes(Lpad, wb, V.T());
    if (P.smem > 48 * 1024)
        (void)hipFuncSetAttribute((const void*)P.kern, hipFuncAttributeMaxDynamicSharedMemorySize, P.smem);
    P.per_cu = 1;
    if (hipOccupancyMaxActiveBlocksPerMultiprocessor(&P.per_cu, (const void*)P.kern, V.T(), (size_t)P.smem) != hipSuccess || P.per_cu < 1)
        P.per_cu = 1;
    P.want_slots = std::min<int64_t>((int64_t)P.work.size(), (int64_t)h->num_cu * P.per_cu);
}

static int sample_clock(const LaunchPlan& P, const PlanRes& R) {
    unsigned long long cyc = 0, ticks = 0;
    const int64_t step = std::max<int64_t>(1, P.n_slots / 24);
    for (int64_t sl = 0; sl < P.n_slots; sl += step) {
        unsigned long long v[10];
        if (hipMemcpy(v, R.arena.as<uint8_t>() + (size_t)sl * P.lay.total + P.lay.hdr + 64, sizeof(v), hipMemcpyDeviceToHost) != hipSuccess) return 0;
        if (v[9] <= v[8] || v[7] <= v[6]) continue;
        cyc += v[7] - v[6];
        ticks += v[9] - v[8];
    }
    return ticks ? (int)((double)cyc / (double)ticks * 100.0 + 0.5) : 0;
}

static int launch_plan(sxg_poa_handle* h, LaunchPlan& P, PlanRes& R, const int prio_base) {
    const Variant V = P.variant;
    int rc;
    if (!P.kern) return fail(SXG_E_INVALID, P.why);
    if ((rc = R.arena.ensure((size_t)P.n_slots * P.lay.total))) return rc;
    {
        const int64_t ns = P.n_slots, ncu = std::max(h->num_cu, 1);
        const int64_t rem = ns % ncu, full = ns / ncu;
        if (rem > 0 && full >= 1 && (int64_t)P.work.size() >= ns) {
            std::vector<int32_t> first((size_t)ns, -1);
            size_t next = 0;
            for (int64_t p = 0; p < ns; ++p)
                if (p % ncu >= rem && p / ncu < full) first[(size_t)p] = P.work[next++];
            for (int64_t round = 0; round <= full; ++round)
                for (int64_t c = 0; c < rem; ++c) {
                    const int64_t cu = (round & 1) ? rem - 1 - c : c, p = round * ncu + cu;
                    if (p < ns && first[(size_t)p] < 0) first[(size_t)p] = P.work[next++];
                }
            std::copy(first.begin(), first.end(), P.work.begin());
        }
    }
    if ((rc = R.work.ensure(4 * P.work.size())) || (rc = R.queue.ensure(256)) || (rc = R.est.ensure(8 * P.work.size()))) return rc;
    HIPCHK(hipMemcpyAsync(R.work.p, P.work.data(), 4 * P.work.size(), hipMemcpyHostToDevice, R.stream));
    P.est.resize(P.work.size());
    for (size_t k = 0; k < P.work.size(); ++k) P.est[k] = (unsigned long long)std::max(h->meta[P.work[k]].cost, 1.0);
    HIPCHK(hipMemcpyAsync(R.est.p, P.est.data(), 8 * P.est.size(), hipMemcpyHostToDevice, R.stream));
    HIPCHK(hipMemsetAsync(R.queue.p, 0, 256, R.stream));
    BlockArgs A;
    A.blk_off = h->d_blk_off.as<int32_t>(); A.seq_off = h->d_seq_off.as<int64_t>(); A.bases = h->d_bases.as<uint8_t>();
    A.weights = h->has_weights ? h->d_weights.as<uint32_t>() : nullptr;
    A.params = h->d_params.as<sxg_poa_params>(); A.per_block_params = h->per_block_params;
    A.work = R.work.as<int32_t>(); A.n_work = (int)P.work.size(); A.queue = R.queue.as<int32_t>();
    A.arena = R.arena.as<uint8_t>(); A.lay = P.lay;
    A.status = h->d_status.as<int32_t>(); A.n_nodes = h->d_nn.as<int32_t>(); A.n_edges = h->d_ne.as<int32_t>();
    A.n_cons = h->d_nc.as<int32_t>(); A.node_code = h->d_node_code.as<uint8_t>();
    A.node_rank = h->d_node_rank.as<int32_t>(); A.node_group = h->d_node_group.as<int32_t>();
    A.edge_tail = h->d_edge_tail.as<int32_t>(); A.edge_head = h->d_edge_head.as<int32_t>();
    A.edge_weight = h->d_edge_w.as<uint32_t>(); A.paths = h->d_paths.as<int32_t>(); A.score = h->d_score.as<int32_t>();
    A.cells = h->d_cells.as<unsigned long long>(); A.cons_nodes = h->d_cons.as<int32_t>();
    A.want_consensus = h->want_consensus;
    A.park_in_lds = P.park_lds ? 1 : 0;
    A.pf_off = P.pf_off;
    A.num_cu = std::max(h->num_cu, 1);
    A.prio_board = getenv("SXG_POA_NO_BALANCE") ? nullptr : h->d_board.as<uint32_t>();
    A.prio_base = prio_base;
    A.est = R.est.as<unsigned long long>();
    A.blk_cycles = h->d_blk_cycles.as<unsigned long long>();
    A.lds_bytes = getenv("SXG_POA_RESORT_NO_LDS") ? 0 : P.smem;
    band_adapt_args(A);
    A.twin = twin_enabled() ? 1 : 0;
    HIPCHK(hipMemset2DAsync(R.arena.as<uint8_t>() + P.lay.hdr, P.lay.total, 0, 512, (size_t)P.n_slots, R.stream));
    HIPCHK(hipStreamWaitEvent(R.stream, h->ev0, 0));
    HIPCHK(hipEventRecord(R.e0, R.stream));
    hipLaunchKernelGGL(P.kern, dim3((unsigned)P.n_slots), dim3(V.T()), (size_t)P.smem, R.stream, A);
    HIPCHK(hipGetLastError());
    HIPCHK(hipEventRecord(R.e1, R.stream));
    HIPCHK(hipStreamWaitEvent(h->stream, R.e1, 0));
    return SXG_OK;
}

static int width_stats_of(const LaunchPlan& P, const PlanRes& R, sxg_poa_width_stats& w, sxg_poa_twin_stats* tw = nullptr) {
    if (P.variant.RM != 2 || P.n_slots <= 0) return SXG_OK;
    constexpr int K0 = 27, K1 = 56;
    std::vector<unsigned long long> v((size_t)P.n_slots * (K1 - K0));
    HIPCHK(hipMemcpy2D(v.data(), (K1 - K0) * 8, R.arena.as<uint8_t>() + P.lay.hdr + 64 + K0 * 8, P.lay.total, (K1 - K0) * 8, (size_t)P.n_slots, hipMemcpyDeviceToHost));
    for (int64_t sl = 0; sl < P.n_slots; ++sl) {
        const unsigned long long* c = v.data() + (size_t)sl * (K1 - K0);
        w.hint_shift_repeats += c[27 - K0];
        for (int k = 0; k < 2; ++k) { w.sweeps[k] += c[49 + k - K0]; w.swept_cols[k] += c[51 + k - K0]; w.swept_cells[k] += c[53 + k - K0]; }
        if (tw) { tw->twin_steps += c[55 - K0] & 0xffffffffull; tw->join_rows += c[55 - K0] >> 32; }
    }
    return SXG_OK;
}

static int debug_plan(sxg_poa_handle* h, LaunchPlan& P, PlanRes& R, int attempt) {
    const Variant V = P.variant;
    unsigned long long acc[8] = {0}, smin = ~0ull, smax = 0;
    for (int64_t sl = 0; sl < P.n_slots; ++sl) {
        unsigned long long one[8];
        HIPCHK(hipMemcpy(one, R.arena.as<uint8_t>() + (size_t)sl * P.lay.total + P.lay.hdr + 64, 64, hipMemcpyDeviceToHost));
        for (int k = 0; k < 8; ++k) acc[k] += one[k];
        unsigned long long st = 0;
        for (int k = 0; k < 6; ++k) st += one[k];
        smin = std::min(smin, st); smax = std::max(smax, st);
    }
    if (V.RM == 2) {
        unsigned long long rep = 0, wsum = 0, nsw = 0;
        for (int64_t sl = 0; sl < P.n_slots; ++sl) {
            unsigned long long v[49];
            HIPCHK(hipMemcpy(v, R.arena.as<uint8_t>() + (size_t)sl * P.lay.total + P.lay.hdr + 64, sizeof(v), hipMemcpyDeviceToHost));
            rep += v[27]; wsum += v[47]; nsw += v[48];
        }
        fprintf(stderr, "[sxg]   band: %llu sweeps, mean width %.1f strips of %d (%.0f columns), %llu hint-shift repeats\n", nsw,
                (double)wsum / (double)std::max(nsw, 1ull), P.lay.band_strips, (double)wsum / (double)std::max(nsw, 1ull) * V.W, rep);
        sxg_poa_width_stats w{};
        sxg_poa_twin_stats tw{};
        if (int rcw = width_stats_of(P, R, w, &tw)) return rcw;
        fprintf(stderr, "[sxg]   width: W=%d %llu sweeps %llu columns %.4g cells; W2=%d %llu sweeps %llu columns %.4g cells\n", V.W, (unsigned long long)w.sweeps[0],
                (unsigned long long)w.swept_cols[0], (double)w.swept_cells[0], P.lay.W2, (unsigned long long)w.sweeps[1], (unsigned long long)w.swept_cols[1], (double)w.swept_cells[1]);
        fprintf(stderr, "[sxg]   twin: %llu twin steps, %llu join rows\n", (unsigned long long)tw.twin_steps, (unsigned long long)tw.join_rows);
    }
    if (const char* path = getenv("SXG_POA_SLOT_CSV")) {
        if (FILE* f = fopen(path, "a")) {
            for (int64_t sl = 0; sl < P.n_slots; ++sl) {
                unsigned long long v[26];
                HIPCHK(hipMemcpy(v, R.arena.as<uint8_t>() + (size_t)sl * P.lay.total + P.lay.hdr + 64, sizeof(v), hipMemcpyDeviceToHost));
                fprintf(f, "%lld,%llu,%llu", (long long)sl, v[8], v[9]);
                for (int w = 0; w < V.NW && w < 16; ++w) fprintf(f, ",%llx", v[10 + w]);
                fprintf(f, "\n");
            }
            fclose(f);
        }
    }
#ifdef SXG_ROW_PROF
    {
        unsigned long long ra[13] = {0};
        for (int64_t sl = 0; sl < P.n_slots; ++sl) {
            unsigned long long one[13];
            HIPCHK(hipMemcpy(one, R.arena.as<uint8_t>() + (size_t)sl * P.lay.total + P.lay.hdr + 64 + 28 * 8, sizeof(one), hipMemcpyDeviceToHost));
            for (int k = 0; k < 13; ++k) ra[k] += one[k];
        }
        double rt = 1e-9;
        for (int k = 0; k < 8; ++k) rt += (double)ra[k];
        static const char* seg16[8] = {"setup", "pass1+scan", "wait left wave", "combine+pass2", "wait right wave", "hand-over+end cell", "stored row fetch", "outgoing+row store"};
        static const char* segb[8] = {"descriptor+band", "predecessor fetch+fold", "pass1+scan+pass2", "end cell+best-cell search", "outgoing+band stores", "-", "-", "-"};
        const char* const* seg = V.RM == 3 ? segb : seg16;
        fprintf(stderr, "[sxg]   row profile:");
        for (int k = 0; k < 8; ++k) fprintf(stderr, " %s %.1f%%", seg[k], 100.0 * (double)ra[k] / rt);
        fprintf(stderr, "\n");
// ... 168 lines not shown
    }
    const int64_t total = h->msa_off_h[(size_t)nb];
    if ((rc = h->d_msa.ensure((size_t)std::max<int64_t>(total, 16) + 16))) return rc;
    if (!items.empty()) {
        if ((rc = h->d_msa_items.ensure(sizeof(MsaItem) * items.size()))) return rc;
        HIPCHK(hipMemcpyAsync(h->d_msa_off.p, h->msa_off_h.data(), 8 * ((size_t)nb + 1), hipMemcpyHostToDevice, h->stream));
        HIPCHK(hipMemcpyAsync(h->d_msa_items.p, items.data(), sizeof(MsaItem) * items.size(), hipMemcpyHostToDevice, h->stream));
        MsaRowsArgs R;
        R.blk_off = C.blk_off; R.seq_off = C.seq_off; R.paths = C.paths; R.cons = C.cons; R.node_code = h->d_node_code.as<uint8_t>();
        R.nn = C.nn; R.nc = C.nc; R.trim = C.trim; R.col = C.col; R.node_o = C.node_o; R.be = C.be; R.msa_off = h->d_msa_off.as<int64_t>();
        R.items = h->d_msa_items.as<MsaItem>(); R.n_items = (int64_t)items.size();
        R.msa = h->d_msa.as<char>(); R.msa_bytes = total;
        const int slots_r = (int)std::min<int64_t>((int64_t)items.size(), (int64_t)h->num_cu * 8);
        HIPCHK(hipEventRecord(h->ev0, h->stream));
        sxg_msa_launch_rows(R, slots_r, h->stream);
        HIPCHK(hipGetLastError());
        HIPCHK(hipEventRecord(h->ev1, h->stream));
        HIPCHK(hipStreamSynchronize(h->stream));
        { float ms = 0; HIPCHK(hipEventElapsedTime(&ms, h->ev0, h->ev1)); h->msa_rows_ms = ms; }
    }
    h->msa_done = true;
    return SXG_OK;
}

extern "C" void sxg_poa_msa_geometry(int32_t* chunk_letters, int32_t* tile_bytes) {
    if (chunk_letters) *chunk_letters = SXG_MSA_CHUNK;
    if (tile_bytes) *tile_bytes = SXG_MSA_TILE;
}

extern "C" int sxg_poa_get_msa_stats(sxg_poa_handle* h, double* cols_ms, double* rows_ms, uint64_t* msa_bytes) {
    if (!h) return fail(SXG_E_INVALID, "handle is NULL");
    if (cols_ms) *cols_ms = h->msa_cols_ms;
    if (rows_ms) *rows_ms = h->msa_rows_ms;
    if (msa_bytes) *msa_bytes = h->msa_done && !h->msa_off_h.empty() ? (uint64_t)h->msa_off_h.back() : 0;
    return SXG_OK;
}

extern "C" int sxg_poa_batch_execute(sxg_poa_handle* h) {
    if (!h) return fail(SXG_E_INVALID, "handle is NULL");
    if (!h->have_batch) return fail(SXG_E_INVALID, "no batch uploaded");
    HIPCHK(hipSetDevice(h->device));
    const RoctxRange range_("sxg_poa_batch_execute");
    h->stats = sxg_poa_stats{};
    h->wstats = sxg_poa_width_stats{};
    h->tstats = sxg_poa_twin_stats{};
    const bool dbg = getenv("SXG_POA_DEBUG") != nullptr;
    auto T0 = std::chrono::steady_clock::now();
    auto lap = [&](const char* what) {
        if (!dbg) return;
        auto T1 = std::chrono::steady_clock::now();
        fprintf(stderr, "[sxg] host %-18s %.3f ms\n", what, std::chrono::duration<double, std::milli>(T1 - T0).count());
        T0 = T1;
    };
    const int nb = h->n_blocks;
    std::vector<int32_t> status(std::max(nb, 1), 0);
    float ms_total = 0;
    std::vector<int32_t> pending;
    for (int b = 0; b < nb; ++b) {
        if (!h->meta[b].fits) status[b] = ST_TOO_LONG; else pending.push_back(b);
    }
    if (nb) HIPCHK(hipMemcpyAsync(h->d_status.p, status.data(), 4 * (size_t)nb, hipMemcpyHostToDevice, h->stream));
    if (nb) {
        HIPCHK(hipMemsetAsync(h->d_nn.p, 0, 4 * (size_t)nb, h->stream));
        HIPCHK(hipMemsetAsync(h->d_ne.p, 0, 4 * (size_t)nb, h->stream));
        HIPCHK(hipMemsetAsync(h->d_nc.p, 0, 4 * (size_t)nb, h->stream));
        HIPCHK(hipMemsetAsync(h->d_blk_cycles.p, 0, 8 * (size_t)nb, h->stream));
    }
    lap("setup");
    std::vector<LaunchPlan> all_plans;
    std::vector<int32_t> nomem_blocks;
    for (int b = 0; b < nb; ++b) h->meta[b].tier = 0;
    for (int attempt = 0; attempt < 7 && !pending.empty(); ++attempt) {
        std::vector<LaunchPlan> plans;
        for (int b : pending) {
            const BlockMeta& m = h->meta[b];
            LaunchPlan* pl = nullptr;
            for (auto& q : plans)
                if (q.variant == m.variant && q.cvx == m.cvx && q.sw == m.sw && q.tier == m.tier && q.wide_band == m.wide_band) { pl = &q; break; }
            if (!pl) { plans.emplace_back(); pl = &plans.back(); pl->variant = m.variant; pl->cvx = m.cvx; pl->sw = m.sw; pl->tier = m.tier; pl->wide_band = m.wide_band; }
            pl->work.push_back(b);
        }
        std::sort(plans.begin(), plans.end(), [](const LaunchPlan& a, const LaunchPlan& b) { return a.variant.Lpad() > b.variant.Lpad(); });
        const double merge_env = getenv("SXG_POA_MERGE") ? atof(getenv("SXG_POA_MERGE")) : 0.0;
        const bool merge_w2 = getenv("SXG_POA_MERGE_WIDTH2") && atoi(getenv("SXG_POA_MERGE_WIDTH2")) != 0 && width2_enabled();
        for (size_t i = 0; i < plans.size(); ++i)
            for (size_t j = i + 1; j < plans.size();) {
                const LaunchPlan &a = plans[i], &b = plans[j];
                const bool join_w2 = merge_w2 && a.variant.NW == b.variant.NW && b.variant.W == class_w2(CLASS_BLOCK, a.variant, a.sw);
                if (same_kind(a.variant, b.variant) && a.variant.RM != 3 && a.cvx == b.cvx && a.sw == b.sw && a.tier == b.tier && a.wide_band == b.wide_band &&
                    (join_w2 || (double)b.variant.Lpad() >= (merge_env > 0 ? merge_env : (a.variant.Lpad() >= 4096 ? 0.92 : 0.75)) * (double)a.variant.Lpad())) {
                    plans[i].work.insert(plans[i].work.end(), b.work.begin(), b.work.end());
                    plans.erase(plans.begin() + (long)j);
                } else ++j;
            }
        if (!getenv("SXG_POA_NO_SPREAD")) {
            uint64_t waves = 0;
            for (auto& pl : plans) waves += (uint64_t)pl.work.size() * (uint64_t)pl.variant.NW;
            for (auto& pl : plans) {
                Variant& v = pl.variant;
                while (v.RM == 2 && v.NW <= 2 && v.W % 2 == 0 && v.W / 2 >= 4 && 2 * waves <= (uint64_t)h->num_cu * 16u) {
                    waves += (uint64_t)pl.work.size() * (uint64_t)v.NW;
                    v = Variant{v.W / 2, 2 * v.NW, class_tmax(v.W / 2, 2 * v.NW, 2, v.CB, true), 2, v.CB, v.DS};
                }
            }
        }
        const uint64_t budget = arena_budget(h);
        uint64_t want_bytes = 0;
        for (auto& pl : plans) {
            std::stable_sort(pl.work.begin(), pl.work.end(), [&](int a, int b) { return h->meta[a].cost > h->meta[b].cost; });
            prepare_plan(h, pl, pl.tier);
            want_bytes += (uint64_t)pl.want_slots * pl.lay.total;
        }
        for (size_t i = 0; i < plans.size();) {
            if ((uint64_t)plans[i].lay.total > budget && plans[i].wide_band) {
                for (int b : plans[i].work) { h->meta[b].wide_band = false; h->meta[b].no_wide = true; }
                plans.erase(plans.begin() + (long)i);
            } else if ((uint64_t)plans[i].lay.total > budget) {
                for (int b : plans[i].work) status[b] = plans[i].tier >= 2 ? ST_POOL_OVERFLOW : ST_ROWS_OVERFLOW;
                g_err = "memory budget too small for a block arena of " + std::to_string(plans[i].lay.total) + " bytes";
                nomem_blocks.insert(nomem_blocks.end(), plans[i].work.begin(), plans[i].work.end());
                plans.erase(plans.begin() + (long)i);
            } else ++i;
        }
        std::vector<double> pcost(plans.size(), 0.0);
        for (size_t i = 0; i < plans.size(); ++i)
            for (int b : plans[i].work)
                pcost[i] += std::max(h->meta[b].cost, 1.0) * (plans[i].variant.RM == 3 ? 1.0 : (double)plans[i].variant.Lpad() / (double)std::max(h->meta[b].maxlen, 1));
        const int oversub = getenv("SXG_POA_OVERSUB") ? std::max(1, atoi(getenv("SXG_POA_OVERSUB"))) : 2;
        auto slots_at = [&](size_t i, double lambda) {
            const double s = lambda * pcost[i] / (double)plans[i].variant.NW;
            return (int64_t)std::min<double>((double)plans[i].want_slots, std::max(1.0, std::floor(s)));
        };
        auto fits = [&](double lambda) {
            uint64_t bytes = 0, waves = 0;
            for (size_t i = 0; i < plans.size(); ++i) {
                const int64_t n = slots_at(i, lambda);
                bytes += (uint64_t)n * plans[i].lay.total;
                waves += (uint64_t)n * (uint64_t)plans[i].variant.NW;
            }
            return bytes <= budget && (plans.size() == 1 || waves <= (uint64_t)h->num_cu * 16u * (uint64_t)oversub);
        };
        double lam_lo = 0.0, lam_hi = 1.0;
        while (lam_hi < 1e30 && fits(lam_hi)) {
            bool all_full = true;
            for (size_t i = 0; i < plans.size(); ++i) all_full = all_full && slots_at(i, lam_hi) >= plans[i].want_slots;
            if (all_full) break;
            lam_hi *= 2.0;
        }
        if (!fits(lam_hi))
            for (int it = 0; it < 100; ++it) {
                const double mid = 0.5 * (lam_lo + lam_hi);
                if (fits(mid)) lam_lo = mid; else lam_hi = mid;
            }
        const double lambda = fits(lam_hi) ? lam_hi : lam_lo;
        (void)want_bytes;
        while (h->planres.size() < plans.size()) {
            PlanRes* r = new PlanRes();
            HIPCHK(hipStreamCreateWithFlags(&r->stream, hipStreamNonBlocking));
            HIPCHK(hipEventCreate(&r->e0));
            HIPCHK(hipEventCreate(&r->e1));
            h->planres.push_back(r);
        }
        for (size_t i = 0; i < plans.size(); ++i) plans[i].n_slots = slots_at(i, lambda);
        lap("plan");
        {
            const size_t board_bytes = (size_t)PRIO_BOARD_CUS * PRIO_BOARD_SLOTS * 4;
            int rcb = h->d_board.ensure(board_bytes);
            if (rcb) return rcb;
            HIPCHK(hipMemsetAsync(h->d_board.p, 0, board_bytes, h->stream));
        }
        HIPCHK(hipEventRecord(h->ev0, h->stream));
        int prio_base = 0;
        for (size_t i = 0; i < plans.size(); ++i) {
            int rc = launch_plan(h, plans[i], *h->planres[i], prio_base);
            if (rc) return rc;
            prio_base += (int)((plans[i].n_slots + h->num_cu - 1) / std::max(h->num_cu, 1));
        }
        HIPCHK(hipEventRecord(h->ev1, h->stream));
        if (attempt == 0 && h->want_block_graph && h->pins && h->n_bases >= ((int64_t)16 << 20) && !getenv("SXG_POA_NO_PINNED")) {
            if (h->pin_thread.joinable()) h->pin_thread.join();
            try {
                h->pin_thread = std::thread([pool = h->pins, dev = h->device, bytes = 4 * (size_t)h->n_bases] {
                    if (hipSetDevice(dev) == hipSuccess) pool->prewarm(bytes);
                });
            } catch (...) {}
        }
        HIPCHK(hipStreamSynchronize(h->stream));
        float ms = 0;
        HIPCHK(hipEventElapsedTime(&ms, h->ev0, h->ev1));
        ms_total += ms;
        for (size_t i = 0; i < plans.size(); ++i) {
            HIPCHK(hipEventElapsedTime(&plans[i].ms, h->planres[i]->e0, h->planres[i]->e1));
            plans[i].clock_mhz = sample_clock(plans[i], *h->planres[i]);
            h->stats.dp_launches += 1;
            h->stats.n_slots += (int)plans[i].n_slots;
            h->stats.device_bytes += (uint64_t)plans[i].n_slots * plans[i].lay.total;
            if (int rcw = width_stats_of(plans[i], *h->planres[i], h->wstats, &h->tstats)) return rcw;
            if (dbg) debug_plan(h, plans[i], *h->planres[i], attempt);
        }
        lap("launches");
        {
            std::vector<int32_t> dev(std::max(nb, 1));
            HIPCHK(hipMemcpy(dev.data(), h->d_status.p, 4 * (size_t)nb, hipMemcpyDeviceToHost));
            for (auto& pl : plans) for (int b : pl.work) status[b] = dev[b];
        }
        std::vector<int32_t> again;
        if (dbg) {
            int cnt[16] = {0};
            for (int b : pending) cnt[status[b] & 15]++;
            fprintf(stderr, "[sxg] round %d: ok %d rows %d pool %d steps %d nodes %d long %d range %d band %d\n", attempt, cnt[0], cnt[1], cnt[2], cnt[3],
                    cnt[4], cnt[5], cnt[6], cnt[7]);
        }
        for (int b : pending) {
            BlockMeta& m = h->meta[b];
            if (std::find(nomem_blocks.begin(), nomem_blocks.end(), b) != nomem_blocks.end()) continue;
            if (status[b] == ST_ROWS_OVERFLOW || status[b] == ST_POOL_OVERFLOW || status[b] == ST_TBX_OVERFLOW || status[b] == ST_NODES_OVERFLOW) {
                if (m.tier < 3) { m.tier += 1; again.push_back(b); }
            } else if (status[b] == ST_BAND_MISS && m.rm == 2 && !m.wide_band && !m.no_wide) {
                m.wide_band = true;
                again.push_back(b);
            } else if (status[b] == ST_RANGE_OVERFLOW || status[b] == ST_BAND_MISS) {
                if (m.rm != 1) {
                    classify_block(m, m.rm >= 2 ? 0 : 1, false);
                    if (m.fits) again.push_back(b);
                    else status[b] = ST_TOO_LONG;
                } else status[b] = ST_TOO_LONG;
            }
        }
        h->stats.retries += (int)again.size();
        pending.swap(again);
        for (auto& pl : plans) all_plans.push_back(std::move(pl));
    }
    for (int b : pending) status[b] = ST_POOL_OVERFLOW;
    if (nb) HIPCHK(hipMemcpy(h->d_status.p, status.data(), 4 * (size_t)nb, hipMemcpyHostToDevice));
    lap("status");
    std::vector<unsigned long long> cells((size_t)std::max<int64_t>(h->n_seqs, 1));
    if (h->n_seqs) HIPCHK(hipMemcpy(cells.data(), h->d_cells.p, 8 * (size_t)h->n_seqs, hipMemcpyDeviceToHost));
    uint64_t total = 0, bytes = 0;
    std::vector<uint64_t> blk_cells(std::max(nb, 1), 0), blk_bytes(std::max(nb, 1), 0);
    for (int b = 0; b < nb; ++b) {
        if (status[b] != ST_OK) continue;
        uint64_t cb = 0;
        for (int s = h->h_blk_off[b]; s < h->h_blk_off[b + 1]; ++s) cb += cells[s];
        const BlockMeta& m = h->meta[b];
        const int ncross = m.S.convex ? 3 : (m.S.g == m.S.e ? 1 : 2);
        const int sz = m.rm == 1 ? 4 : 2;
        blk_cells[b] = cb; blk_bytes[b] = cb * (uint64_t)(2 * ncross * sz + 1);
        total += cb;
        bytes += blk_bytes[b];
    }
    for (auto& pl : all_plans) {
        for (int b : pl.work) if (status[b] == ST_OK) { pl.cells += blk_cells[b]; pl.bytes += blk_bytes[b]; }
// ... 1720 lines not shown
```

### smoothxg_amd/poa.py

```python
import ctypes as C
import os

import numpy as np

from . import build as _build

MODE_LOCAL, MODE_GLOBAL = 0, 1


class Params(C.Structure):
    _fields_ = [("m", C.c_int8), ("n", C.c_int8), ("g", C.c_int8), ("e", C.c_int8),
                ("q", C.c_int8), ("c", C.c_int8), ("mode", C.c_uint8), ("banded", C.c_uint8)]


def params_from_cli(m=1, n=4, g=6, e=2, q=26, c=1, local=True):
    return Params(m, -n, -g, -e, -q, -c, MODE_LOCAL if local else MODE_GLOBAL, 0)


_i32p, _i64p, _u8p, _u32p, _u64p = (C.POINTER(C.c_int32), C.POINTER(C.c_int64), C.POINTER(C.c_uint8),
                                    C.POINTER(C.c_uint32), C.POINTER(C.c_uint64))


class BatchIn(C.Structure):
    _fields_ = [("n_blocks", C.c_int32), ("blk_off", _i32p), ("seq_off", _i64p), ("bases", _u8p),
# ... 2 lines not shown
                ("want_block_graph", C.c_int32), ("bg_consensus_visited_only", C.c_int32), ("bg_trim", _i32p)]


class BatchOut(C.Structure):
    _fields_ = [("n_blocks", C.c_int32), ("n_seqs", C.c_int64), ("status", _i32p), ("node_off", _i64p),
                ("node_code", _u8p), ("node_rank", _i32p), ("node_group", _i32p), ("edge_off", _i64p),
                ("edge_tail", _i32p), ("edge_head", _i32p), ("edge_weight", _u32p),
                ("seq_path_nodes", _i32p), ("score", _i32p), ("cells", _u64p), ("cons_off", _i64p),
                ("cons_nodes", _i32p), ("msa_off", _i64p), ("msa_cols", _i32p), ("msa", C.c_void_p),
                ("bg_node_off", _i64p), ("bg_node_len", _i32p), ("bg_node_outdeg", _i32p), ("bg_node_indeg", _u8p),
                ("bg_seq_off", _i64p), ("bg_seq", C.c_void_p), ("bg_edge_off", _i64p), ("bg_edge_to", _i32p),
                ("bg_step_off", _i64p), ("bg_steps", _i32p), ("bg_cons_off", _i64p), ("bg_cons_steps", _i32p),
                ("block_cycles", _u64p), ("_owner", C.c_void_p)]


class AlignIn(C.Structure):
    _fields_ = [("n", C.c_int32), ("row_off", _i64p), ("row_code", _u8p), ("row_sink", _u8p),
                ("pred_off", _i64p), ("preds", _i32p), ("seq_off", _i64p), ("bases", _u8p),
                ("params", C.POINTER(Params)), ("per_problem_params", C.c_int32)]


class AlignOut(C.Structure):
    _fields_ = [("n", C.c_int32), ("status", _i32p), ("score", _i32p), ("pair_off", _i64p),
                ("pair_row", _i32p), ("pair_pos", _i32p), ("_owner", C.c_void_p)]


class Stats(C.Structure):
    _fields_ = [("kernel_ms", C.c_double), ("cells", C.c_uint64), ("dp_launches", C.c_uint64),
                ("algo_bytes", C.c_uint64), ("n_slots", C.c_int32), ("retries", C.c_int32),
                ("device_bytes", C.c_uint64), ("dom_kernel_ms", C.c_double), ("dom_cells", C.c_uint64),
                ("dom_algo_bytes", C.c_uint64), ("dom_threads", C.c_int32), ("dom_cols_per_lane", C.c_int32),
                ("dom_row_mode", C.c_int32), ("dom_clock_mhz", C.c_int32), ("bg_ms", C.c_double)]


class WidthStats(C.Structure):
    _fields_ = [("sweeps", C.c_uint64 * 2), ("swept_cols", C.c_uint64 * 2), ("swept_cells", C.c_uint64 * 2),
                ("hint_shift_repeats", C.c_uint64), ("dom_width", C.c_int32), ("dom_width2", C.c_int32)]


class TwinStats(C.Structure):
    _fields_ = [("twin_steps", C.c_uint64), ("join_rows", C.c_uint64)]


class DeviceView(C.Structure):
    _fields_ = [("n_blocks", C.c_int32), ("n_seqs", C.c_int64), ("n_bases", C.c_int64),
                ("status", C.c_void_p), ("n_nodes", C.c_void_p), ("n_edges", C.c_void_p),
                ("node_code", C.c_void_p), ("node_rank", C.c_void_p), ("node_group", C.c_void_p),
                ("edge_tail", C.c_void_p), ("edge_head", C.c_void_p), ("edge_weight", C.c_void_p),
                ("seq_path_nodes", C.c_void_p), ("score", C.c_void_p)]


class SplitIn(C.Structure):
    _fields_ = [("n_blocks", C.c_int32), ("blk_off", _i32p), ("seq_off", _i64p), ("bases", _u8p),
                ("identity", C.POINTER(C.c_double)), ("length_ratio_min", C.POINTER(C.c_double))]


class SplitOut(C.Structure):
    _fields_ = [("n_blocks", C.c_int32), ("n_seqs", C.c_int64), ("group", _i32p), ("n_groups", _i32p),
                ("n_pairs", _i64p), ("status", _i32p), ("_owner", C.c_void_p)]


class SplitMash(C.Structure):
    _fields_ = [("kmer_size", C.c_int32), ("min_len", _i32p), ("est_identity", C.POINTER(C.c_double))]


class IdentityIn(C.Structure):
    _fields_ = [("n_blocks", C.c_int32), ("blk_off", _i32p), ("seq_off", _i64p), ("bases", _u8p), ("kmer_size", C.c_int32),
                ("min_len", C.c_int32), ("percentile", C.c_double)]


class SgdIn(C.Structure):
    _fields_ = [("n_nodes", C.c_int64), ("node_len", _i32p), ("n_paths", C.c_int64), ("path_off", _i64p), ("step_node", _i32p),
                ("step_pos", _i64p), ("iter_max", C.c_int32), ("cooling_start", C.c_int32), ("eta", C.POINTER(C.c_double)),
                ("terms_per_iter", C.c_uint64), ("seed", C.c_uint64), ("mode", C.c_int32)]


SGD_LDS_NODES = 8192
MASH_SORT_TILE = 1024
SPLIT_PANEL = 512
MAX_SEQ_LEN = 26623
ST_TOO_LONG = 5
MSA_FULL, MSA_TRIMMED = 1, 2

EXPORTS = ["sxg_poa_block_identity_batch", "sxg_poa_path_sgd_order", "sxg_poa_kmer_jaccard_batch", "sxg_poa_split_mash_batch", "sxg_poa_pair_identity_batch", "sxg_poa_split_batch", "sxg_poa_split_free", "sxg_poa_batch_device_view", "sxg_poa_abi_version", "sxg_poa_device_count", "sxg_poa_last_error", "sxg_poa_create",
           "sxg_poa_destroy", "sxg_poa_batch_run", "sxg_poa_batch_upload", "sxg_poa_batch_execute",
           "sxg_poa_batch_download", "sxg_poa_batch_free", "sxg_poa_align_batch", "sxg_poa_align_free",
           "sxg_poa_get_stats", "sxg_poa_get_width_stats", "sxg_poa_get_twin_stats", "sxg_poa_set_memory_budget", "sxg_xxh64", "sxg_poa_comm_unique_id", "sxg_poa_comm_init",
           "sxg_poa_comm_attach", "sxg_poa_comm_destroy", "sxg_poa_batch_run_sharded", "sxg_poa_batch_run_sharded_local",
           "sxg_poa_batch_upload_sharded", "sxg_poa_batch_execute_sharded", "sxg_poa_batch_download_sharded", "sxg_poa_sharded_info",
           "sxg_poa_sharded_timing", "sxg_poa_measure_copy", "sxg_poa_roctx_available", "sxg_poa_get_msa_stats", "sxg_poa_msa_geometry"]
COMM_ID_BYTES = 128
NOT_ROOT = 1

_lib = None


def load_library(build_if_missing=True):
    global _lib
    if _lib is not None:
        return _lib
    so = os.environ.get("SXG_POA_LIB", _build.SO)
    if not os.path.exists(so):
        if not build_if_missing:
            raise RuntimeError("libsxgpoa.so is missing: run `python -m smoothxg_amd.build`")
        _build.build()
    L = C.CDLL(so)
    vp = C.c_void_p
    L.sxg_poa_last_error.restype = C.c_char_p
    L.sxg_poa_create.argtypes = [C.c_int, C.POINTER(vp)]
    L.sxg_poa_destroy.argtypes = [vp]
    L.sxg_poa_batch_run.argtypes = [vp, C.POINTER(BatchIn), C.POINTER(BatchOut)]
    L.sxg_poa_batch_upload.argtypes = [vp, C.POINTER(BatchIn)]
    L.sxg_poa_batch_execute.argtypes = [vp]
    L.sxg_poa_batch_download.argtypes = [vp, C.POINTER(BatchOut)]
    L.sxg_poa_batch_free.argtypes = [C.POINTER(BatchOut)]
    L.sxg_poa_batch_device_view.argtypes = [vp, C.POINTER(DeviceView)]
    L.sxg_poa_align_batch.argtypes = [vp, C.POINTER(AlignIn), C.POINTER(AlignOut)]
    L.sxg_poa_align_free.argtypes = [C.POINTER(AlignOut)]
    L.sxg_poa_get_stats.argtypes = [vp, C.POINTER(Stats)]
    L.sxg_poa_get_width_stats.argtypes = [vp, C.POINTER(WidthStats)]
    L.sxg_poa_get_twin_stats.argtypes = [vp, C.POINTER(TwinStats)]
    L.sxg_poa_set_memory_budget.argtypes = [vp, C.c_uint64]
    L.sxg_poa_get_msa_stats.argtypes = [vp, C.POINTER(C.c_double), C.POINTER(C.c_double), C.POINTER(C.c_uint64)]
    L.sxg_poa_msa_geometry.argtypes = [C.POINTER(C.c_int32), C.POINTER(C.c_int32)]
    L.sxg_poa_msa_geometry.restype = None
    L.sxg_poa_measure_copy.argtypes = [vp, C.c_uint64, C.c_int, C.POINTER(C.c_double)]
    L.sxg_poa_comm_unique_id.argtypes = [C.POINTER(C.c_uint8)]
    L.sxg_poa_comm_init.argtypes = [vp, C.POINTER(C.c_uint8), C.c_int, C.c_int]
    L.sxg_poa_comm_attach.argtypes = [vp, vp, C.c_int, C.c_int]
    L.sxg_poa_comm_destroy.argtypes = [vp]
    L.sxg_poa_comm_destroy.restype = None
    L.sxg_poa_batch_run_sharded.argtypes = [vp, C.POINTER(BatchIn), C.POINTER(BatchOut)]
    L.sxg_poa_batch_run_sharded_local.argtypes = [vp, C.POINTER(BatchIn), C.c_int, C.POINTER(BatchOut)]
    L.sxg_poa_batch_upload_sharded.argtypes = [vp, C.POINTER(BatchIn)]
    L.sxg_poa_batch_execute_sharded.argtypes = [vp]
    L.sxg_poa_batch_download_sharded.argtypes = [vp, C.POINTER(BatchIn), C.POINTER(BatchOut)]
    L.sxg_poa_sharded_info.argtypes = [vp, C.POINTER(C.c_int32), C.POINTER(C.c_uint64)]
    L.sxg_poa_sharded_timing.argtypes = [vp, C.POINTER(C.c_double), C.POINTER(C.c_double)]
    L.sxg_poa_pair_identity_batch.argtypes = [vp, C.c_int64, _i64p, _u8p, C.c_int64, _i32p, _i32p, _u8p, _i32p, _i32p, _i32p, _i32p]
    L.sxg_poa_split_batch.argtypes = [vp, C.POINTER(SplitIn), C.POINTER(SplitOut)]
    L.sxg_poa_split_free.argtypes = [C.POINTER(SplitOut)]
    L.sxg_poa_kmer_jaccard_batch.argtypes = [vp, C.c_int64, _i64p, _u8p, C.c_int32, C.c_int64, _i32p, _i32p, _i32p, _i32p, C.POINTER(C.c_uint64)]
    L.sxg_poa_split_mash_batch.argtypes = [vp, C.POINTER(SplitIn), C.POINTER(SplitMash), C.POINTER(SplitOut), _i64p]
    L.sxg_poa_split_free.restype = None
    L.sxg_poa_block_identity_batch.argtypes = [vp, C.POINTER(IdentityIn), _i32p, _i32p, _i32p, _i32p]
    L.sxg_poa_path_sgd_order.argtypes = [vp, C.POINTER(SgdIn), _i32p, _i64p]
    L.sxg_xxh64.restype = C.c_uint64
    L.sxg_xxh64.argtypes = [C.c_char_p, C.c_uint64, C.c_uint64]
    _lib = L
    return L


class PoaError(RuntimeError):
    pass


def _p(a, t):
    return a.ctypes.data_as(C.POINTER(t))


def _arr(ptr, n, dtype):
    if n == 0 or not ptr:
        return np.zeros(0, dtype)
    return np.ctypeslib.as_array(ptr, shape=(n,)).astype(dtype, copy=True)


class BlockResult:
    __slots__ = ("status", "node_code", "node_rank", "node_group", "edge_tail", "edge_head", "edge_weight",
                 "paths", "scores", "cells", "consensus", "msa", "bg", "device_cycles")


class BlockGraph:
    __slots__ = ("node_seq", "node_indeg", "edges", "paths", "consensus")

    def gfa(self, names, revs=None, consensus_name=None):
        o = ["H\tVN:Z:1.0"]
        o += ["S\t%d\t%s" % (i + 1, s) for i, s in enumerate(self.node_seq)]
        o += ["L\t%d\t+\t%d\t+\t0M" % (a + 1, b + 1) for a, b in self.edges]
        for i, p in enumerate(self.paths):
            for j, nm in enumerate(names[i]):
                st = ["%d-" % (v + 1) for v in p[::-1]] if revs is not None and revs[i][j] else ["%d+" % (v + 1) for v in p]
                o.append("P\t%s\t%s\t*" % (nm, ",".join(st)))
        if consensus_name is not None:
            o.append("P\t%s\t%s\t*" % (consensus_name, ",".join("%d+" % (v + 1) for v in self.consensus)))
        return "\n".join(o) + "\n"


class PoaEngine:

    def __init__(self, device=0):
        self.lib = load_library()
        if self.lib.sxg_poa_device_count() <= 0:
            raise PoaError("no HIP device: the blocked-POA engine has no CPU fallback")
        h = C.c_void_p()
        rc = self.lib.sxg_poa_create(device, C.byref(h))
        if rc:
            raise PoaError("sxg_poa_create: %s" % self.lib.sxg_poa_last_error().decode())
        self.h = h
        self._keep = None
        self._shape = None

    def close(self):
        if getattr(self, "h", None):
            self.lib.sxg_poa_destroy(self.h)
            self.h = None

    def __del__(self):
        try:
            self.close()
        except Exception:
            pass

    def _err(self, what):
        return PoaError("%s: %s" % (what, self.lib.sxg_poa_last_error().decode()))

    def set_memory_budget(self, nbytes):
        self.lib.sxg_poa_set_memory_budget(self.h, int(nbytes))

    def _mk_in(self, bases, seq_off, blk_off, weights, params, want_consensus, want_msa, block_graph=0, bg_trim=None,
               bg_cons_visited_only=False):
        bases = np.ascontiguousarray(bases, np.uint8)
        seq_off = np.ascontiguousarray(seq_off, np.int64)
        blk_off = np.ascontiguousarray(blk_off, np.int32)
        nb = len(blk_off) - 1
        if isinstance(params, Params):
            parr = (Params * 1)(params)
            per = 0
        else:
            parr = (Params * max(len(params), 1))(*params)
            per = 1
        w = None if weights is None else np.ascontiguousarray(weights, np.uint32)
        bpad = bases if len(bases) else np.zeros(1, np.uint8)
        trim = None if bg_trim is None else np.ascontiguousarray(bg_trim, np.int32)
        bi = BatchIn(nb, _p(blk_off, C.c_int32), _p(seq_off, C.c_int64), _p(bpad, C.c_uint8),
                     _p(w, C.c_uint32) if w is not None else None, parr, per, int(want_consensus),
                     int(want_msa), int(block_graph), int(bool(bg_cons_visited_only)),
                     _p(trim, C.c_int32) if trim is not None else None)
        self._keep = (bpad, seq_off, blk_off, w, parr, trim)
        return bi

    def upload(self, bases, seq_off, blk_off, weights, params, want_consensus=False, want_msa=False, block_graph=0,
               bg_trim=None, bg_cons_visited_only=False):
        bi = self._mk_in(bases, seq_off, blk_off, weights, params, want_consensus, want_msa, block_graph, bg_trim,
                         bg_cons_visited_only)
        if self.lib.sxg_poa_batch_upload(self.h, C.byref(bi)):
            raise self._err("sxg_poa_batch_upload")
        self._shape = (np.asarray(blk_off).copy(), np.asarray(seq_off).copy(), int(want_msa))

    def execute(self, check=True):
        rc = self.lib.sxg_poa_batch_execute(self.h)
        if rc and (check or rc != -4):
            raise self._err("sxg_poa_batch_execute")
        return rc

    def stats(self):
        s = Stats()
        self.lib.sxg_poa_get_stats(self.h, C.byref(s))
        st = {f[0]: getattr(s, f[0]) for f in Stats._fields_}
        w = WidthStats()
        self.lib.sxg_poa_get_width_stats(self.h, C.byref(w))
        st.update(width_sweeps=tuple(w.sweeps), width_swept_cols=tuple(w.swept_cols), width_swept_cells=tuple(w.swept_cells),
                  hint_shift_repeats=w.hint_shift_repeats, dom_width=w.dom_width, dom_width2=w.dom_width2)
        tw = TwinStats()
        self.lib.sxg_poa_get_twin_stats(self.h, C.byref(tw))
        st.update(twin_steps=tw.twin_steps, join_rows=tw.join_rows)
        return st

    def msa_geometry(self):
        a, b = C.c_int32(), C.c_int32()
        self.lib.sxg_poa_msa_geometry(C.byref(a), C.byref(b))
        return a.value, b.value

    def msa_stats(self):
        a, b, n = C.c_double(), C.c_double(), C.c_uint64()
        self.lib.sxg_poa_get_msa_stats(self.h, C.byref(a), C.byref(b), C.byref(n))
        return a.value, b.value, n.value

    def device_view(self):
        v = DeviceView()
        if self.lib.sxg_poa_batch_device_view(self.h, C.byref(v)):
            raise self._err("sxg_poa_batch_device_view")
        return v

    def download(self):
        out = BatchOut()
        if self.lib.sxg_poa_batch_download(self.h, C.byref(out)):
            raise self._err("sxg_poa_batch_download")
        try:
            return self._unpack(out)
        finally:
            self.lib.sxg_poa_batch_free(C.byref(out))

    def _unpack(self, out, shape=None):
        shape = shape if shape is not None else self._shape
        blk_off, seq_off = shape[:2]
        msa_mode = shape[2] if len(shape) > 2 else 0
        nb = out.n_blocks
        ns = int(out.n_seqs)
        status = _arr(out.status, nb, np.int32)
        node_off = _arr(out.node_off, nb + 1, np.int64)
        edge_off = _arr(out.edge_off, nb + 1, np.int64)
        nn, ne = (int(node_off[-1]), int(edge_off[-1])) if nb else (0, 0)
        has_raw = bool(out.node_code) or nn == 0
        node_code = _arr(out.node_code, nn, np.uint8) if has_raw else None
        node_rank = _arr(out.node_rank, nn, np.int32) if has_raw else None
        node_group = _arr(out.node_group, nn, np.int32) if has_raw else None
        et = _arr(out.edge_tail, ne, np.int32) if has_raw else None
        eh = _arr(out.edge_head, ne, np.int32) if has_raw else None
        ew = _arr(out.edge_weight, ne, np.uint32) if has_raw else None
        nbases = int(seq_off[-1]) if ns else 0
        paths = _arr(out.seq_path_nodes, nbases, np.int32) if out.seq_path_nodes else None
        bg = None
        if out.bg_node_off:
            bno = _arr(out.bg_node_off, nb + 1, np.int64)
            bso = _arr(out.bg_seq_off, nb + 1, np.int64)
            beo = _arr(out.bg_edge_off, nb + 1, np.int64)
            bpo = _arr(out.bg_step_off, ns + 1, np.int64)
            bg = dict(no=bno, so=bso, eo=beo, po=bpo, ln=_arr(out.bg_node_len, int(bno[-1]), np.int32),
                      od=_arr(out.bg_node_outdeg, int(bno[-1]), np.int32), idg=_arr(out.bg_node_indeg, int(bno[-1]), np.uint8),
                      sq=C.string_at(out.bg_seq, int(bso[-1])) if bso[-1] else b"", to=_arr(out.bg_edge_to, int(beo[-1]), np.int32),
                      st=_arr(out.bg_steps, int(bpo[-1]), np.int32))
            if out.bg_cons_off:
                bg["co"] = _arr(out.bg_cons_off, nb + 1, np.int64)
                bg["cs"] = _arr(out.bg_cons_steps, int(bg["co"][-1]), np.int32)
        score = _arr(out.score, ns, np.int32)
        cells = _arr(out.cells, ns, np.uint64)
        cycles = _arr(out.block_cycles, nb, np.uint64) if out.block_cycles else None
        cons_off = _arr(out.cons_off, nb + 1, np.int64) if out.cons_off else None
        cons = _arr(out.cons_nodes, int(cons_off[-1]), np.int32) if cons_off is not None and nb and out.cons_nodes else None
        msa_off = _arr(out.msa_off, nb + 1, np.int64) if out.msa_off else None
        msa_cols = _arr(out.msa_cols, nb, np.int32) if out.msa_cols else None
        msa_raw = None
        if msa_off is not None and nb and msa_off[-1] > 0:
            msa_raw = C.string_at(out.msa, int(msa_off[-1]))
        res = []
        for b in range(nb):
            r = BlockResult()
            r.status = int(status[b])
            a, z = node_off[b], node_off[b + 1]
            r.node_code, r.node_rank, r.node_group = (node_code[a:z], node_rank[a:z], node_group[a:z]) if has_raw else (None, None, None)
            a, z = edge_off[b], edge_off[b + 1]
            r.edge_tail, r.edge_head, r.edge_weight = (et[a:z], eh[a:z], ew[a:z]) if has_raw else (None, None, None)
            s0, s1 = int(blk_off[b]), int(blk_off[b + 1])
            r.paths = [paths[int(seq_off[s]):int(seq_off[s + 1])] for s in range(s0, s1)] if paths is not None else None
            r.bg = None
            if bg is not None:
                g = BlockGraph()
                a, z = int(bg["no"][b]), int(bg["no"][b + 1])
                ln, od = bg["ln"][a:z], bg["od"][a:z]
# ... 276 lines not shown
```

Baseline: 707.9.

## Use variant-aware block cost model for scheduling, slot sizing and priority balancing

Adds a per-block cost model that uses the actual padded column width of each launch variant and growing graph size. The model drives work sorting, slot allocation across plans, and the remaining-work estimate fed to the in-kernel priority board, which now reads precomputed per-sequence progress. Balance progress is now counted in padded columns rather than sequence length. Width-2 merging is enabled by default when enough packed work exists to fill the CUs. The aim is better load balance and less tail imbalance, with the risk that the heuristic mis-ranks blocks and adds host work plus an extra upload.

```diff
diff --git a/include/sxg_poa.h b/include/sxg_poa.h
--- a/include/sxg_poa.h
+++ b/include/sxg_poa.h
@@ -150,6 +150,7 @@
 int sxg_poa_measure_copy(sxg_poa_handle *h, uint64_t bytes, int reps, double *gbps);
 int sxg_poa_roctx_available(void);
 int sxg_poa_device_count(void);
+int sxg_poa_compute_units(sxg_poa_handle *h);
 const char *sxg_poa_last_error(void);
 
 int sxg_poa_create(int device, sxg_poa_handle **out);
diff --git a/smoothxg_amd/build.py b/smoothxg_amd/build.py
--- a/smoothxg_amd/build.py
+++ b/smoothxg_amd/build.py
@@ -7,7 +7,7 @@
 KERN_PARTS = range(1, 10)
 SOURCES = [("sxg_poa.hip", "sxg_poa.o", []), ("kern_split.hip", "kern_split.o", []), ("kern_msa.hip", "kern_msa.o", []),
            ("kern_sgd.hip", "kern_sgd.o", ["-ffp-contract=off"])] + [("kern_part.hip", "kern_part%d.o" % k, ["-DSXG_KERN_PART=%d" % k]) for k in KERN_PARTS]
-DEPS = ["sxg_poa.hip", "kern_part.hip", "poa_classes.h", "poa_kernels.hip.h", "poa_kern_tables.hip.h", "poa_dp.hip.h", "poa_dp16.hip.h", "poa_dp16_fill.inc.h", "poa_dp16_row.inc.h", "poa_prep_rows.inc.h", "poa_rowcode.h", "poa_band16.hip.h", "poa_graph_dev.h",
+DEPS = ["sxg_poa.hip", "kern_part.hip", "poa_classes.h", "poa_cost.h", "poa_kernels.hip.h", "poa_kern_tables.hip.h", "poa_dp.hip.h", "poa_dp16.hip.h", "poa_dp16_fill.inc.h", "poa_dp16_row.inc.h", "poa_prep_rows.inc.h", "poa_rowcode.h", "poa_band16.hip.h", "poa_graph_dev.h",
                   "poa_bgraph_dev.h", "poa_types.h", "kern_split.hip", "poa_split.hip.h", "poa_mash.hip.h", "poa_identity.hip.h", "poa_identity_key.h", "kern_sgd.hip", "poa_sgd.hip.h", "kern_msa.hip", "poa_msa.hip.h", "poa_msa_cols.h", os.path.join("..", "..", "include", "sxg_poa.h")]
 OBJ_DIR = os.path.join(CSRC, "build")
 
diff --git a/smoothxg_amd/csrc/poa_band16.hip.h b/smoothxg_amd/csrc/poa_band16.hip.h
--- a/smoothxg_amd/csrc/poa_band16.hip.h
+++ b/smoothxg_amd/csrc/poa_band16.hip.h
@@ -1,19 +1,16 @@
 #pragma once
 #include <hip/hip_runtime.h>
 #include "poa_dp16.hip.h"
+#include "poa_cost.h"
 
 namespace sxg {
 
-constexpr int BAND_WB = 311;
-constexpr double BAND_WF = 0.03;
 constexpr int BAND_W_MAX = 11;
 constexpr int BAND_WIN = 128;
-constexpr int BAND_WMAX = 693;
 __host__ __device__ inline int band_strip_width(int maxlen) {
     const int w0 = BAND_WB + (int)(BAND_WF * maxlen), w = w0 < BAND_WMAX ? w0 : BAND_WMAX;
     return 2 * w <= 756 ? 6 : (2 * w <= 1008 ? 8 : 11);
 }
-__host__ __device__ inline int band_half_width(int L) { const int w = BAND_WB + (int)(BAND_WF * L); return w < BAND_WMAX ? w : BAND_WMAX; }
 __host__ __device__ inline int band_plane_strips(int maxlen, int W) { return plane_round4(2 * band_half_width(maxlen) / W + 2); }
 __host__ __device__ constexpr int band_lds_bytes(int W) { return LDS_CTL_BYTES + LDS_META_BYTES / 2 + 64 * W * 8; }
 
diff --git a/smoothxg_amd/csrc/poa_cost.h b/smoothxg_amd/csrc/poa_cost.h
--- /dev/null
+++ b/smoothxg_amd/csrc/poa_cost.h
@@ -0,0 +1,51 @@
+#pragma once
+#include <stdint.h>
+
+#include <cstddef>
+#include <vector>
+
+#include "poa_classes.h"
+
+namespace sxg {
+
+constexpr int BAND_WB = 311;
+constexpr double BAND_WF = 0.03;
+constexpr int BAND_WMAX = 693;
+constexpr int band_half_width(int L) { const int w = BAND_WB + (int)(BAND_WF * L); return w < BAND_WMAX ? w : BAND_WMAX; }
+
+constexpr uint64_t cost_cols(int rm, int T, int W, int W2, int64_t len) {
+    if (rm == 3) return 2u * (uint64_t)band_half_width((int)len);
+    if (rm == 2) return (uint64_t)T * 2u * (uint64_t)width_for_len(W, W2, T, (int)len);
+    return (uint64_t)T * (uint64_t)W;
+}
+
+inline uint64_t block_cost(const int64_t* off, int n, int rm, int T, int W, int W2, uint64_t* done) {
+    uint64_t total = 0;
+    double prev = 0;
+    const double l0 = n > 0 ? (double)(off[1] - off[0]) : 0.0;
+    for (int k = 0; k < n; ++k) {
+        const int64_t len = off[k + 1] - off[k];
+        if (done) done[k] = total;
+        if (k > 0) total += (uint64_t)((l0 + 0.05 * prev) * (double)cost_cols(rm, T, W, W2, len));
+        prev += (double)len;
+    }
+    return total;
+}
+
+inline void deal_over_cus(std::vector<int32_t>& work, int64_t ns, int64_t ncu) {
+    if (ncu < 1) ncu = 1;
+    const int64_t rem = ns % ncu, full = ns / ncu;
+    if (rem <= 0 || full < 1 || (int64_t)work.size() < ns) return;
+    std::vector<int32_t> first((size_t)ns, -1);
+    size_t next = 0;
+    for (int64_t p = 0; p < ns; ++p)
+        if (p % ncu >= rem && p / ncu < full) first[(size_t)p] = work[next++];
+    for (int64_t round = 0; round <= full; ++round)
+        for (int64_t c = 0; c < rem; ++c) {
+            const int64_t cu = (round & 1) ? rem - 1 - c : c, p = round * ncu + cu;
+            if (p < ns && first[(size_t)p] < 0) first[(size_t)p] = work[next++];
+        }
+    for (int64_t p = 0; p < ns; ++p) work[(size_t)p] = first[(size_t)p];
+}
+
+}
diff --git a/smoothxg_amd/csrc/poa_dp.hip.h b/smoothxg_amd/csrc/poa_dp.hip.h
--- a/smoothxg_amd/csrc/poa_dp.hip.h
+++ b/smoothxg_amd/csrc/poa_dp.hip.h
@@ -294,7 +294,7 @@
     const int kL = L - j0;
 
     for (int i = 1; i <= N; ++i) {
-        if (B.prio_board) { if ((i & 127) == 1) sxg_balance_prio(B, (unsigned long long)i * (unsigned long long)L); }
+        if (B.prio_board) { if ((i & 127) == 1) sxg_balance_prio(B, (unsigned long long)i * (unsigned long long)Lpad); }
         else if ((i & 63) == 1) sxg_rotate_prio(B.prio_rank);
         const int r = i - 1;
         if ((r & (META_CHUNK - 1)) == 0) {
diff --git a/smoothxg_amd/csrc/poa_dp16_fill.inc.h b/smoothxg_amd/csrc/poa_dp16_fill.inc.h
--- a/smoothxg_amd/csrc/poa_dp16_fill.inc.h
+++ b/smoothxg_amd/csrc/poa_dp16_fill.inc.h
@@ -171,7 +171,7 @@
     i32x8 dnext = cmeta[0];
     if constexpr (TWIN) { const int d1_ = dnext[1]; asm volatile("" :: "s"(d1_)); }
     for (int i = 1; i <= N; ++i) {
-        if (has_board) { if ((i & 127) == 1) sxg_balance_prio(B, (unsigned long long)i * (unsigned long long)L); }
+        if (has_board) { if ((i & 127) == 1) sxg_balance_prio(B, (unsigned long long)i * (unsigned long long)(2 * TW)); }
         else if ((i & 63) == 1) sxg_rotate_prio(prio_rank);
         i32x8 dsc = dnext;
         dnext = cmeta[min(i, N - 1)];
@@ -234,7 +234,7 @@
             while (flags & ROW_TWIN) {
                 if (has_board) {
                     const int due = ((i + 1) & 127) == 1 ? i + 1 : ((((i + 2) & 127) == 1 && i + 2 <= N) ? i + 2 : 0);
-                    if (due) sxg_balance_prio(B, (unsigned long long)due * (unsigned long long)L);
+                    if (due) sxg_balance_prio(B, (unsigned long long)due * (unsigned long long)(2 * TW));
                 } else if (((i + 1) & 63) == 1 || (((i + 2) & 63) == 1 && i + 2 <= N)) sxg_rotate_prio(prio_rank);
                 if (p0 != i - 1) {
                     int hl;
diff --git a/smoothxg_amd/csrc/poa_kernels.hip.h b/smoothxg_amd/csrc/poa_kernels.hip.h
--- a/smoothxg_amd/csrc/poa_kernels.hip.h
+++ b/smoothxg_amd/csrc/poa_kernels.hip.h
@@ -171,6 +171,7 @@
     uint32_t* prio_board;
     int prio_base;
     const unsigned long long* est;
+    const unsigned long long* est_done;
     int lds_bytes;
     unsigned long long* blk_cycles;
     int band_floor, band_margin, band_full;
@@ -205,7 +206,6 @@
         if (wi >= A.n_work) break;
         const int b = A.work[wi];
         const unsigned long long est_total = A.est ? A.est[wi] : 0ull;
-        unsigned long long done_cells = 0;
         const int s0 = A.blk_off[b], s1 = A.blk_off[b + 1];
         const int64_t base0 = A.seq_off[s0];
         const Scoring S = normalise(A.params[A.per_block_params ? b : 0]);
@@ -253,7 +253,8 @@
                 if (status != ST_OK) break;
                 PROF(1);
                 DpResult res;
-                V.B.prio_rem0 = est_total > done_cells ? est_total - done_cells : 0ull;
+                const unsigned long long done_cost = A.est_done ? A.est_done[s] : 0ull;
+                V.B.prio_rem0 = est_total > done_cost ? est_total - done_cost : 0ull;
                 if constexpr (RM == 3) {
                     V.B.band_w = band_half_width(len);
                     V.B.band_mode = band_mode;
@@ -334,7 +335,6 @@
                 score = res.bi >= 0 ? res.best : 0;
             }
             if (t == 0) { A.score[s] = score; if (RM != 3 || N == 0 || len == 0) A.cells[s] = RM == 3 ? 0ull : (unsigned long long)N * (unsigned long long)len; }
-            done_cells += (unsigned long long)N * (unsigned long long)len;
             const bool spoa_order = (A.params[A.per_block_params ? b : 0].mode & SXG_ORDER_SPOA) != 0;
             if (CT.graph_batch == 16 || (CT.graph_batch == 8 && T <= 64)) { WgCtxT<16> c16{ctx.lds}; add_alignment(c16, V.G, seq, len, A.weights ? A.weights[s] : 1u, A.paths + so, !spoa_order); }
             else if (CT.graph_batch == 8) { WgCtxT<8> c8{ctx.lds}; add_alignment(c8, V.G, seq, len, A.weights ? A.weights[s] : 1u, A.paths + so, !spoa_order); }
diff --git a/smoothxg_amd/csrc/sxg_poa.hip b/smoothxg_amd/csrc/sxg_poa.hip
--- a/smoothxg_amd/csrc/sxg_poa.hip
+++ b/smoothxg_amd/csrc/sxg_poa.hip
@@ -16,6 +16,7 @@
 #include <rccl/rccl.h>
 #include <dlfcn.h>
 #include "poa_kernels.hip.h"
+#include "poa_cost.h"
 #include "poa_kern_tables.hip.h"
 #include "poa_split.hip.h"
 #include "poa_mash.hip.h"
@@ -271,6 +272,8 @@
         d_paths, d_score, d_cells, d_cons, d_work, d_queue, d_arena, d_blk_cycles;
     DevBuf d_tmp_a, d_tmp_b, d_tmp_c, d_tmp_d;
     DevBuf d_board;
+    std::vector<uint64_t> blk_cost, seq_done;
+    DevBuf d_est_done;
     int want_block_graph = 0, bg_cons_visited_only = 0;
     std::shared_ptr<PinPool> pins;
     std::thread pin_thread;
@@ -366,6 +369,7 @@
     { std::lock_guard<std::mutex> lk(g_err_mu); g_err_ret = g_err_any; }
     return g_err_ret.c_str();
 }
+extern "C" int sxg_poa_compute_units(sxg_poa_handle* h) { return h ? h->num_cu : -1; }
 extern "C" int sxg_poa_device_count(void) {
     int n = 0;
     if (hipGetDeviceCount(&n) != hipSuccess) return 0;
@@ -397,7 +401,7 @@
     DevBuf* bufs[] = {&h->d_blk_off, &h->d_seq_off, &h->d_bases, &h->d_weights, &h->d_params, &h->d_status, &h->d_nn,
                       &h->d_ne, &h->d_nc, &h->d_node_code, &h->d_node_rank, &h->d_node_group, &h->d_edge_tail,
                       &h->d_edge_head, &h->d_edge_w, &h->d_paths, &h->d_score, &h->d_cells, &h->d_cons, &h->d_work,
-                      &h->d_queue, &h->d_arena, &h->d_blk_cycles, &h->d_tmp_a, &h->d_tmp_b, &h->d_tmp_c, &h->d_tmp_d, &h->d_board, &h->d_trim, &h->d_bg_no, &h->d_bg_eo,
+                      &h->d_queue, &h->d_arena, &h->d_blk_cycles, &h->d_tmp_a, &h->d_tmp_b, &h->d_tmp_c, &h->d_tmp_d, &h->d_board, &h->d_est_done, &h->d_trim, &h->d_bg_no, &h->d_bg_eo,
                       &h->d_bg_len, &h->d_bg_od, &h->d_bg_id, &h->d_bg_seq, &h->d_bg_eto, &h->d_bg_steps, &h->d_bg_nsteps, &h->d_bg_cons,
                       &h->d_bg_counts, &h->d_bg_work, &h->d_bg_queue, &h->d_bg_arena,
                       &h->d_msa_no, &h->d_msa_tmp, &h->d_msa_col, &h->d_msa_be, &h->d_msa_off, &h->d_msa_items, &h->d_msa_work, &h->d_msa_queue, &h->d_msa};
@@ -667,26 +671,11 @@
     int rc;
     if (!P.kern) return fail(SXG_E_INVALID, P.why);
     if ((rc = R.arena.ensure((size_t)P.n_slots * P.lay.total))) return rc;
-    {
-        const int64_t ns = P.n_slots, ncu = std::max(h->num_cu, 1);
-        const int64_t rem = ns % ncu, full = ns / ncu;
-        if (rem > 0 && full >= 1 && (int64_t)P.work.size() >= ns) {
-            std::vector<int32_t> first((size_t)ns, -1);
-            size_t next = 0;
-            for (int64_t p = 0; p < ns; ++p)
-                if (p % ncu >= rem && p / ncu < full) first[(size_t)p] = P.work[next++];
-            for (int64_t round = 0; round <= full; ++round)
-                for (int64_t c = 0; c < rem; ++c) {
-                    const int64_t cu = (round & 1) ? rem - 1 - c : c, p = round * ncu + cu;
-                    if (p < ns && first[(size_t)p] < 0) first[(size_t)p] = P.work[next++];
-                }
-            std::copy(first.begin(), first.end(), P.work.begin());
-        }
-    }
+    deal_over_cus(P.work, P.n_slots, std::max(h->num_cu, 1));
     if ((rc = R.work.ensure(4 * P.work.size())) || (rc = R.queue.ensure(256)) || (rc = R.est.ensure(8 * P.work.size()))) return rc;
     HIPCHK(hipMemcpyAsync(R.work.p, P.work.data(), 4 * P.work.size(), hipMemcpyHostToDevice, R.stream));
     P.est.resize(P.work.size());
-    for (size_t k = 0; k < P.work.size(); ++k) P.est[k] = (unsigned long long)std::max(h->meta[P.work[k]].cost, 1.0);
+    for (size_t k = 0; k < P.work.size(); ++k) P.est[k] = (unsigned long long)std::max<uint64_t>(h->blk_cost[(size_t)P.work[k]], 1);
     HIPCHK(hipMemcpyAsync(R.est.p, P.est.data(), 8 * P.est.size(), hipMemcpyHostToDevice, R.stream));
     HIPCHK(hipMemsetAsync(R.queue.p, 0, 256, R.stream));
     BlockArgs A;
@@ -708,6 +697,7 @@
     A.prio_board = getenv("SXG_POA_NO_BALANCE") ? nullptr : h->d_board.as<uint32_t>();
     A.prio_base = prio_base;
     A.est = R.est.as<unsigned long long>();
+    A.est_done = h->d_est_done.as<unsigned long long>();
     A.blk_cycles = h->d_blk_cycles.as<unsigned long long>();
     A.lds_bytes = getenv("SXG_POA_RESORT_NO_LDS") ? 0 : P.smem;
     band_adapt_args(A);
@@ -1042,7 +1032,13 @@
         }
         std::sort(plans.begin(), plans.end(), [](const LaunchPlan& a, const LaunchPlan& b) { return a.variant.Lpad() > b.variant.Lpad(); });
         const double merge_env = getenv("SXG_POA_MERGE") ? atof(getenv("SXG_POA_MERGE")) : 0.0;
-        const bool merge_w2 = getenv("SXG_POA_MERGE_WIDTH2") && atoi(getenv("SXG_POA_MERGE_WIDTH2")) != 0 && width2_enabled();
+        bool merge_w2 = width2_enabled();
+        if (const char* e = getenv("SXG_POA_MERGE_WIDTH2")) merge_w2 = merge_w2 && atoi(e) != 0;
+        else {
+            size_t packed = 0;
+            for (const auto& q : plans) if (q.variant.RM == 2) packed += q.work.size();
+            merge_w2 = merge_w2 && packed >= (size_t)std::max(h->num_cu, 1);
+        }
         for (size_t i = 0; i < plans.size(); ++i)
             for (size_t j = i + 1; j < plans.size();) {
                 const LaunchPlan &a = plans[i], &b = plans[j];
@@ -1066,9 +1062,15 @@
         }
         const uint64_t budget = arena_budget(h);
         uint64_t want_bytes = 0;
+        h->blk_cost.assign((size_t)std::max(nb, 1), 0);
+        h->seq_done.assign((size_t)std::max<int64_t>(h->n_seqs, 1), 0);
         for (auto& pl : plans) {
-            std::stable_sort(pl.work.begin(), pl.work.end(), [&](int a, int b) { return h->meta[a].cost > h->meta[b].cost; });
             prepare_plan(h, pl, pl.tier);
+            const Variant& v = pl.variant;
+            for (int b : pl.work)
+                h->blk_cost[(size_t)b] = block_cost(h->h_seq_off.data() + h->h_blk_off[b], h->h_blk_off[b + 1] - h->h_blk_off[b], v.RM, v.T(), v.W, v.W2,
+                                                    h->seq_done.data() + h->h_blk_off[b]);
+            std::stable_sort(pl.work.begin(), pl.work.end(), [&](int a, int b) { return h->blk_cost[(size_t)a] > h->blk_cost[(size_t)b]; });
             want_bytes += (uint64_t)pl.want_slots * pl.lay.total;
         }
         for (size_t i = 0; i < plans.size();) {
@@ -1084,8 +1086,7 @@
         }
         std::vector<double> pcost(plans.size(), 0.0);
         for (size_t i = 0; i < plans.size(); ++i)
-            for (int b : plans[i].work)
-                pcost[i] += std::max(h->meta[b].cost, 1.0) * (plans[i].variant.RM == 3 ? 1.0 : (double)plans[i].variant.Lpad() / (double)std::max(h->meta[b].maxlen, 1));
+            for (int b : plans[i].work) pcost[i] += (double)std::max<uint64_t>(h->blk_cost[(size_t)b], 1);
         const int oversub = getenv("SXG_POA_OVERSUB") ? std::max(1, atoi(getenv("SXG_POA_OVERSUB"))) : 2;
         auto slots_at = [&](size_t i, double lambda) {
             const double s = lambda * pcost[i] / (double)plans[i].variant.NW;
@@ -1128,6 +1129,8 @@
             int rcb = h->d_board.ensure(board_bytes);
             if (rcb) return rcb;
             HIPCHK(hipMemsetAsync(h->d_board.p, 0, board_bytes, h->stream));
+            if ((rcb = h->d_est_done.ensure(8 * h->seq_done.size()))) return rcb;
+            HIPCHK(hipMemcpyAsync(h->d_est_done.p, h->seq_done.data(), 8 * h->seq_done.size(), hipMemcpyHostToDevice, h->stream));
         }
         HIPCHK(hipEventRecord(h->ev0, h->stream));
         int prio_base = 0;
diff --git a/smoothxg_amd/poa.py b/smoothxg_amd/poa.py
--- a/smoothxg_amd/poa.py
+++ b/smoothxg_amd/poa.py
@@ -108,7 +108,7 @@
 ST_TOO_LONG = 5
 MSA_FULL, MSA_TRIMMED = 1, 2
 
-EXPORTS = ["sxg_poa_block_identity_batch", "sxg_poa_path_sgd_order", "sxg_poa_kmer_jaccard_batch", "sxg_poa_split_mash_batch", "sxg_poa_pair_identity_batch", "sxg_poa_split_batch", "sxg_poa_split_free", "sxg_poa_batch_device_view", "sxg_poa_abi_version", "sxg_poa_device_count", "sxg_poa_last_error", "sxg_poa_create",
+EXPORTS = ["sxg_poa_block_identity_batch", "sxg_poa_path_sgd_order", "sxg_poa_kmer_jaccard_batch", "sxg_poa_split_mash_batch", "sxg_poa_pair_identity_batch", "sxg_poa_split_batch", "sxg_poa_split_free", "sxg_poa_batch_device_view", "sxg_poa_abi_version", "sxg_poa_device_count", "sxg_poa_compute_units", "sxg_poa_last_error", "sxg_poa_create",
            "sxg_poa_destroy", "sxg_poa_batch_run", "sxg_poa_batch_upload", "sxg_poa_batch_execute",
            "sxg_poa_batch_download", "sxg_poa_batch_free", "sxg_poa_align_batch", "sxg_poa_align_free",
            "sxg_poa_get_stats", "sxg_poa_get_width_stats", "sxg_poa_get_twin_stats", "sxg_poa_set_memory_budget", "sxg_xxh64", "sxg_poa_comm_unique_id", "sxg_poa_comm_init",
@@ -143,6 +143,7 @@
     L.sxg_poa_batch_device_view.argtypes = [vp, C.POINTER(DeviceView)]
     L.sxg_poa_align_batch.argtypes = [vp, C.POINTER(AlignIn), C.POINTER(AlignOut)]
     L.sxg_poa_align_free.argtypes = [C.POINTER(AlignOut)]
+    L.sxg_poa_compute_units.argtypes = [vp]
     L.sxg_poa_get_stats.argtypes = [vp, C.POINTER(Stats)]
     L.sxg_poa_get_width_stats.argtypes = [vp, C.POINTER(WidthStats)]
     L.sxg_poa_get_twin_stats.argtypes = [vp, C.POINTER(TwinStats)]
@@ -291,6 +292,9 @@
         self.lib.sxg_poa_get_twin_stats(self.h, C.byref(tw))
         st.update(twin_steps=tw.twin_steps, join_rows=tw.join_rows)
         return st
+
+    def compute_units(self):
+        return int(self.lib.sxg_poa_compute_units(self.h))
 
     def msa_geometry(self):
         a, b = C.c_int32(), C.c_int32()
```

Result: faster. 716.1 (median of 6 runs) (+1.1%).
